# jibo27/3DGS_Hierarchical_Training

Hardware: AMD Instinct MI355X
Metric: train-step images/sec + fwd+bwd ms @1M Gaussians, 980x545; 1/2/4/8 GPU (higher is better)
Workload: dtype f32

## Files before the change

### 3dgs_hierarchical_training_amd/csrc/gsr_kernels.hip

```cpp
#include <hip/hip_runtime.h>
#include <hip/hip_ext.h>
#include <type_traits>
#include <stdint.h>
#include <stdio.h>
#include <string.h>

#include <algorithm>
#include <atomic>
#include <chrono>
#include <cmath>
#include <map>
#include <mutex>
#include <tuple>
#include <vector>

#include "../../include/gsr.h"
#include "gsr_math.h"
#include "adam_math.h"
#include "radix_sort.h"
#include "blend_common.h"

#ifndef GSR_K9_UNROLL
#define GSR_K9_UNROLL 2
#endif
// ... 271 lines not shown
            for (int c = 0; c < 4; c++) {
                s_sh[g * kShStride + col0 + e] = xs[c];
                if (++e == ROW) { e = 0; g++; }
            }
        }
    }
}

template <int ROW, int KN>
__device__ __forceinline__ void stage_store_lin(const float4 (&r)[KN], float* tile, int nG, int tid)
{
    float4* t4 = reinterpret_cast<float4*>(tile);
#pragma unroll
    for (int q = 0; q < stage_regs<ROW>(); q++) {
        const int v = tid + q * kPreThreads;
        if (v < (nG * ROW) / 4) t4[v] = r[q];
    }
}

template <int ROW, int KN>
__device__ __forceinline__ void stage_load_full(float4 (&r)[KN], const float* __restrict__ src, int tid)
{
    static_assert(KN >= stage_regs<ROW>(), "register file too small for the rows");
    constexpr int total4 = kPreThreads * ROW / 4;
    const float4* s4 = reinterpret_cast<const float4*>(src);
#pragma unroll
    for (int q = 0; q < stage_regs<ROW>(); q++) {
        const int v = tid + q * kPreThreads;
        if ((q + 1) * kPreThreads <= total4 || v < total4) r[q] = s4[v];
    }
}
template <int ROW, int KN>
__device__ __forceinline__ void stage_store_lin_full(const float4 (&r)[KN], float* tile, int tid)
{
    constexpr int total4 = kPreThreads * ROW / 4;
    float4* t4 = reinterpret_cast<float4*>(tile);
#pragma unroll
    for (int q = 0; q < stage_regs<ROW>(); q++) {
        const int v = tid + q * kPreThreads;
        if ((q + 1) * kPreThreads <= total4 || v < total4) t4[v] = r[q];
    }
}

__device__ __forceinline__ void count_large_rects(bool act, Splat& s, TileRec& rec, int W, int H, int tiles_x, int tiles_y, int tid)
{
    const int lane = tid & 63;
    for (unsigned long long pm = __ballot(act && s.tiles == kTilesPending); pm != 0ull; pm &= pm - 1ull) {
        const int src = (int)__builtin_ctzll(pm);
        const float bpx = __shfl(s.px, src, 64), bpy = __shfl(s.py, src, 64), bca = __shfl(s.ca, src, 64);
        const float bcb = __shfl(s.cb, src, 64), bcc = __shfl(s.cc, src, 64), bop = __shfl(s.op, src, 64);
        const int brad = __shfl(s.radius, src, 64);
        int x0, y0, x1, y1;
        tile_rect_tight(bpx, bpy, brad, bca, bcb, bcc, bop, W, H, tiles_x, tiles_y, x0, y0, x1, y1);
        const int ww = x1 - x0, full = ww * (y1 - y0);
        const TileTest tt = make_tile_test(bpx, bpy, bca, bcb, bcc, bop);
        uint32_t cnt = 0;
        for (int c0 = 0; c0 < full; c0 += 64) {
            const int c = c0 + lane;
            bool ok = false;
            if (c < full) {
                const int ty = c / ww, tx = c - ty * ww;
                ok = tile_accept(tt, x0 + tx, y0 + ty, W, H);
            }
            cnt += (uint32_t)__popcll(__ballot(ok));
        }
        if (lane == src) { s.tiles = cnt; rec.mask = cnt; }
    }
}

struct DepthHist {
    uint32_t* ghist;
    uint32_t* status;
    uint32_t status_words;
    uint32_t clear_threads;
};

template <int DEG, bool RAW, bool SHO = false>
__global__ __launch_bounds__(kPreThreads) void k_preprocess(CamParams cp, int N, const float* __restrict__ means,
                                                            const float* __restrict__ scales, const float* __restrict__ rots,
                                                            const float* __restrict__ cov_pre, const float* __restrict__ opac,
                                                            const float* __restrict__ shs, const float* __restrict__ shs_rest,
                                                            const float* __restrict__ colors,
                                                            Splat* __restrict__ splat, int32_t* __restrict__ radii,
                                                            uint32_t* __restrict__ dkey, uint32_t* __restrict__ gid,
                                                            TileRec* __restrict__ tilerec, uint32_t* __restrict__ zero_words,
                                                            int zero_count, int block0, DepthHist dh, uint2* __restrict__ early_parts = nullptr,
                                                            uint32_t window_max = 0xffffffffu, uint8_t* __restrict__ visible = nullptr,
                                                            const float* __restrict__ sh_origin = nullptr)
{
    constexpr int NC3 = 3 * (DEG + 1) * (DEG + 1);
    __shared__ float s_sh[kPreThreads * kShStride];
    __shared__ uint32_t s_early[2][kPreThreads / 64];
    const int tid = threadIdx.x;
    const int base = ((int)blockIdx.x + block0) * kPreThreads;
    const int i = base + tid;
    const int model = select_view(cp, (int)blockIdx.x + block0);
    if (blockIdx.x == 0)
        for (int q = tid; q < zero_count; q += kPreThreads) zero_words[q] = 0u;
    constexpr int NR = NC3 > 3 ? NC3 - 3 : 1;
    float4 r_dc[1];
    float4 r_rows[stage_regs<NC3>()];
    bool pend_dc = false, pend_rest = false, pend_full = false;
    const int nG = min(kPreThreads, N - base);
    if (shs) {
        if (shs_rest) {
            const size_t row = (size_t)(cp.M - 1) * 3;
            const float* dc0 = shs + (size_t)base * 3;
            if (vec_ok(dc0, nG * 3)) { stage_load<3>(r_dc, dc0, nG, tid); pend_dc = true; }
            else for (int f = tid; f < nG * 3; f += kPreThreads) s_sh[(f / 3) * kShStride + (f % 3)] = dc0[f];
            if (NC3 > 3) {
                const float* r0 = shs_rest + (size_t)base * row;
                if (row == NR && vec_ok(r0, nG * NR)) { stage_load<NR>(r_rows, r0, nG, tid); pend_rest = true; }
                else for (int f = tid; f < nG * NR; f += kPreThreads) {
                    const int g = f / NR, e = f - g * NR;
                    s_sh[g * kShStride + 3 + e] = shs_rest[(size_t)(base + g) * row + e];
                }
            }
        } else {
            const size_t row = (size_t)cp.M * 3;
            const float* r0 = shs + (size_t)base * row;
            if (row == NC3 && vec_ok(r0, nG * NC3)) { stage_load<NC3>(r_rows, r0, nG, tid); pend_full = true; }
            else for (int f = tid; f < nG * NC3; f += kPreThreads) {
                const int g = f / NC3, e = f - g * NC3;
                s_sh[g * kShStride + e] = shs[(size_t)(base + g) * row + e];
            }
        }
    }
    const bool act = i < N;
    Camera cam = load_camera(cp);
    cam.D = DEG;
    float mean[3] = {0.f, 0.f, 0.f};
    float mraw[3] = {0.f, 0.f, 0.f};
    Splat s;
    TileRec rec;
    uint32_t lo_pack = 0u;
    if (act) {
        mean[0] = means[3 * (size_t)i]; mean[1] = means[3 * (size_t)i + 1]; mean[2] = means[3 * (size_t)i + 2];
        if constexpr (SHO) { mraw[0] = mean[0]; mraw[1] = mean[1]; mraw[2] = mean[2]; }
        apply_points_transform(cp.xf, mean);
        float sc[3] = {0, 0, 0}, rq[4] = {1, 0, 0, 0}, cv[6], colp[3];
        if (cov_pre) {
#pragma unroll
            for (int k = 0; k < 6; k++) cv[k] = cov_pre[6 * (size_t)i + k];
        } else {
#pragma unroll
            for (int k = 0; k < 3; k++) sc[k] = scales[3 * (size_t)i + k];
#pragma unroll
            for (int k = 0; k < 4; k++) rq[k] = rots[4 * (size_t)i + k];
        }
        if (colors) {
#pragma unroll
            for (int k = 0; k < 3; k++) colp[k] = colors[3 * (size_t)i + k];
        }
        float op = opac[i];
        if (RAW) {
            if (!cov_pre) {
#pragma unroll
                for (int k = 0; k < 3; k++) sc[k] = expf(sc[k]);
                const float inv = 1.0f / fmaxf(sqrtf(rq[0] * rq[0] + rq[1] * rq[1] + rq[2] * rq[2] + rq[3] * rq[3]), 1e-12f);
#pragma unroll
                for (int k = 0; k < 4; k++) rq[k] *= inv;
            }
            op = 1.0f / (1.0f + expf(-op));
        }
        preprocess_one(cam, mean, sc, rq, cov_pre ? cv : nullptr, op, nullptr, 3, 1, colors ? colp : nullptr, s, &rec, true, &lo_pack);
    }
    count_large_rects(act, s, rec, cp.W, cp.H, cam.tiles_x, cam.tiles_y, tid);
    rec.rect += (uint32_t)(model * cam.tiles_y) << 12;
    if (early_parts) {
        const uint32_t nt = act ? s.tiles : 0u;
        const uint32_t far = (nt > 0u && __float_as_uint(s.depth) - kDepthKeyBias > window_max) ? 1u : 0u;
        const uint32_t st_ = wave_inclusive_sum(nt), sf_ = wave_inclusive_sum(far);
        if ((tid & 63) == 63) { s_early[0][tid >> 6] = st_; s_early[1][tid >> 6] = sf_; }
        __syncthreads();
        if (tid == 0) {
            uint32_t t0 = 0u, t1 = 0u;
#pragma unroll
            for (int w = 0; w < kPreThreads / 64; w++) { t0 += s_early[0][w]; t1 += s_early[1][w]; }
            early_parts[blockIdx.x + block0] = make_uint2(t0, t1);
        }
    }
    if (shs) {
        constexpr bool kLinOk = NC3 > 3 && (NR & 1);
        const bool lin = kLinOk && pend_dc && pend_rest;
        float* s_dc = s_sh;
        float* s_rest = s_sh + kPreThreads * 3;
        if (lin) {
            stage_store_lin<3>(r_dc, s_dc, nG, tid);
            stage_store_lin<NR>(r_rows, s_rest, nG, tid);
        } else {
            if (pend_dc) stage_store<3>(r_dc, s_sh, 0, nG, tid);
            if (pend_rest) stage_store<NR>(r_rows, s_sh, 3, nG, tid);
            if (pend_full) stage_store<NC3>(r_rows, s_sh, 0, nG, tid);
        }
        __syncthreads();
        if (act && s.radius > 0) {
            float col[3];
            if constexpr (SHO) {
#pragma unroll
                for (int k = 0; k < 3; k++) { cam.cam[k] = sh_origin[k]; mean[k] = mraw[k]; }
            }
            if (lin) splat_sh_color(cam, mean, s_rest + tid * NR - 3, 3, 1, col, s_dc + tid * 3);
            else splat_sh_color(cam, mean, &s_sh[tid * kShStride], 3, 1, col);
            s.r = col[0]; s.g = col[1]; s.b = col[2];
        }
    }
    if (dh.ghist && dh.clear_threads == 0u)
        for (uint32_t q = tid; q < dh.status_words / 4; q += kPreThreads) reinterpret_cast<uint4*>(dh.status)[q] = make_uint4(0u, 0u, 0u, 0u);
    if (!act) return;
    {
        Splat st = s;
        st.tiles = lo_pack;
        splat[i] = st;
    }
    tilerec[i] = rec;
    radii[i] = s.radius;
    if (visible) visible[i] = s.radius > 0 ? 1 : 0;
    const uint32_t key = s.tiles > 0 ? __float_as_uint(s.depth) : 0xffffffffu;
    dkey[i] = key;
    gid[i] = (uint32_t)i;
    if (dh.ghist) {
        const uint32_t x = (uint32_t)i / onesweep_run_len<uint32_t>((uint32_t)N);
#pragma unroll
        for (int p = 0; p < 4; p++) atomicAdd(&dh.ghist[((size_t)p * kOsRanges + x) * 256 + ((key >> (8 * p)) & 255u)], 1u);
    }
}

__global__ __launch_bounds__(256) void k_prepared_begin(int N, const int32_t* __restrict__ radii_in, int32_t* __restrict__ radii_out,
                                                        uint32_t* __restrict__ zero_words, int zero_count)
{
    const int i = blockIdx.x * 256 + threadIdx.x;
    if (i < N) radii_out[i] = radii_in[i];
    if (blockIdx.x == 0)
        for (int q = threadIdx.x; q < zero_count; q += 256) zero_words[q] = 0u;
}

__global__ void k_mark_visible(int N, const float* __restrict__ means, const float* __restrict__ vm, uint8_t* __restrict__ present)
{
    const int i = blockIdx.x * blockDim.x + threadIdx.x;
    if (i >= N) return;
    float v[16];
#pragma unroll
    for (int k = 0; k < 16; k++) v[k] = vm[k];
    present[i] = depth_key(v, means[3 * (size_t)i], means[3 * (size_t)i + 1], means[3 * (size_t)i + 2]) > kNearZ ? 1 : 0;
}

constexpr int kEmitThreads = 256;

__device__ __forceinline__ uint32_t block_inclusive_scan_256(uint32_t v, uint32_t* s_wave , uint32_t& total)
{
    const int lane = threadIdx.x & 63, wave = threadIdx.x >> 6;
    uint32_t x = v;
#pragma unroll
    for (int off = 1; off < 64; off <<= 1) {
        const uint32_t y = __shfl_up(x, off, 64);
        if (lane >= off) x += y;
    }
    if (lane == 63) s_wave[wave] = x;
    __syncthreads();
    uint32_t add = 0;
    for (int w = 0; w < wave; w++) add += s_wave[w];
    total = s_wave[0] + s_wave[1] + s_wave[2] + s_wave[3];
    return x + add;
}

struct ZeroJobs {
    void* p[3];
    uint32_t words[3];
};

__device__ __forceinline__ void scan_report_late(unsigned long long* late_out, unsigned long long all, unsigned long long seq)
{
    __atomic_store_n(late_out, all, __ATOMIC_RELAXED);
    __atomic_store_n(late_out + 2, (unsigned long long)g_onesweep_giveups, __ATOMIC_RELAXED);
    __threadfence_system();
    __atomic_store_n(late_out + 1, seq, __ATOMIC_RELAXED);
    __threadfence_system();
}
template <int NTHR>
__device__ __forceinline__ void block_scan_body(uint32_t* block_sums, int nb, unsigned long long* total_out, const ZeroJobs& zj,
                                                unsigned long long* host_out, unsigned long long host_seq, unsigned long long* s_wsum ,
                                                const unsigned int* window_overflow = nullptr, unsigned long long* late_out = nullptr)
{
    constexpr int NWV = NTHR / 64;
    const int tid = threadIdx.x, lane = tid & 63, wave = tid >> 6;
#pragma unroll
    for (int j = 0; j < 3; j++) {
        uint32_t* z = static_cast<uint32_t*>(zj.p[j]);
        for (uint32_t q = tid; q < zj.words[j]; q += NTHR) z[q] = 0u;
    }
    const int chunk = (nb + NTHR - 1) / NTHR;
    const int lo = min(nb, tid * chunk), hi = min(nb, lo + chunk);
    unsigned long long sum = 0;
    for (int b = lo; b < hi; b++) sum += block_sums[b];
    unsigned long long inc = sum;
#pragma unroll
    for (int off = 1; off < 64; off <<= 1) {
        const unsigned long long y = __shfl_up(inc, off, 64);
        if (lane >= off) inc += y;
    }
    if (lane == 63) s_wsum[wave] = inc;
    __syncthreads();
    unsigned long long add = 0, all = 0;
// ... 1483 lines not shown
        const uint32_t* __restrict__ cur = bb.cur;
        const uint16_t* __restrict__ perm = bb.perm;
        const uint32_t e = cur[0];
        if (table && cur[1 + (blockIdx.x & 7u)]) {
            const int k = (int)perm[blockIdx.x];
            if (k < bb.nslots4) kslot = k;
        }
        if (e < (uint32_t)kVcEntries) cost_out = bb.cost + (size_t)e * bb.items;
    }
}

template <bool REACH>
__global__ __launch_bounds__(64) void k_blend_fwd_w6(int W, int H, int tiles_x, int T, const uint2* __restrict__ ranges,
                                                     const uint32_t* __restrict__ list, const Splat* __restrict__ splat,
                                                     const float* __restrict__ bg, float* __restrict__ out_color,
                                                     float* __restrict__ out_depth, float* __restrict__ out_alpha,
                                                     float* __restrict__ img, uint32_t* __restrict__ staged4, int interleave,
                                                     float* __restrict__ ckpt, int kCkptFirst, int tiles_y, const BlendBalance bb,
                                                     float* __restrict__ out_clamped, const ListCut cut = ListCut{}, const int cut_pass = 0)
{
    if (cut_pass == 2 && cut.ctl[2] == 0u) return;
    __shared__ float4 s_ab[2 * kFwdBufs][64];
    __shared__ float2 s_c[kFwdBufs][64];
    int kslot = (int)(blockIdx.x >> 3);
    uint16_t* cost_out = nullptr;
    blend_fwd_slot(bb, cut_pass != 2, kslot, cost_out);
    blend_fwd_item<REACH>((int)(blockIdx.x & 7), kslot, s_ab, s_c, W, H, tiles_x, T, ranges, list, splat, bg, out_color, out_depth,
                          out_alpha, img, staged4, interleave, ckpt, kCkptFirst, tiles_y, cost_out, out_clamped, cut, cut_pass);
}

template <bool HAS_DA>
__global__ __launch_bounds__(64) void k_blend_fwd_render(int W, int H, int tiles_x, int T, const uint2* __restrict__ ranges,
                                                         const uint32_t* __restrict__ list, const Splat* __restrict__ splat,
                                                         const float* __restrict__ bg, float* __restrict__ out_color,
                                                         float* __restrict__ out_depth, float* __restrict__ out_alpha,
                                                         float* __restrict__, uint32_t* __restrict__, int interleave,
                                                         float* __restrict__, int, int tiles_y, const BlendBalance bb,
                                                         float* __restrict__ out_clamped, const ListCut, const int)
{
    __shared__ float4 s_ab[2 * kFwdBufs][64];
    __shared__ float2 s_c[kFwdBufs][64];
    int kslot = (int)(blockIdx.x >> 3);
    uint16_t* cost_out = nullptr;
    blend_fwd_slot(bb, true, kslot, cost_out);
    blend_fwd_item<true, false, true, HAS_DA>((int)(blockIdx.x & 7), kslot, s_ab, s_c, W, H, tiles_x, T, ranges, list, splat, bg, out_color, out_depth,
                                              out_alpha, nullptr, nullptr, interleave, nullptr, 0, tiles_y, cost_out, out_clamped, ListCut{}, 0);
}

__global__ __launch_bounds__(64) void k_blend_importance(int W, int H, int tiles_x, int T, const uint2* __restrict__ ranges,
                                                         const uint32_t* __restrict__ list, const Splat* __restrict__ splat,
                                                         float* __restrict__ img, uint32_t* __restrict__ staged4, int interleave, int tiles_y,
                                                         const float* __restrict__ color, float* __restrict__ S)
{
    __shared__ float4 s_ab[2 * kFwdBufs][64];
    __shared__ float s_sum[3][64];
    __shared__ uint32_t s_id[64];
    blend_fwd_item<true, true>((int)(blockIdx.x & 7), (int)(blockIdx.x >> 3), s_ab, nullptr, W, H, tiles_x, T, ranges, list, splat, nullptr, nullptr, nullptr,
                               nullptr, img, staged4, interleave, nullptr, 0, tiles_y, nullptr, nullptr, ListCut{}, 0, ImpArgs{color, S, s_sum, s_id});
}

__global__ __launch_bounds__(256) void k_importance_finish(int N, int M, int D, const float* __restrict__ means, const float* __restrict__ xf,
                                                           const float* __restrict__ campos, const float* __restrict__ sh_origin,
                                                           const Splat* __restrict__ splat, const float* __restrict__ S, float* __restrict__ acc)
{
    const int n = (int)blockIdx.x * 16 + (int)(threadIdx.x >> 4), k = (int)(threadIdx.x & 15);
    if (n >= N || k >= (D + 1) * (D + 1)) return;
    const float4 s = reinterpret_cast<const float4*>(S)[n];
    if (s.x == 0.f && s.y == 0.f && s.z == 0.f) return;
    float mean[3] = {means[3 * (size_t)n], means[3 * (size_t)n + 1], means[3 * (size_t)n + 2]};
    float o[3];
    if (sh_origin) { o[0] = sh_origin[0]; o[1] = sh_origin[1]; o[2] = sh_origin[2]; }
    else { apply_points_transform(xf, mean); o[0] = campos[0]; o[1] = campos[1]; o[2] = campos[2]; }
    float basis[16];
    sh_basis_dir(D, mean, o, basis);
    const Splat sp = splat[n];
    const float b = fabsf(basis[k]);
    float* a = acc + ((size_t)n * M + k) * 3;
    if (sp.r > 0.f) a[0] += b * s.x;
    if (sp.g > 0.f) a[1] += b * s.y;
    if (sp.b > 0.f) a[2] += b * s.z;
}


constexpr size_t kItemHdrBytes = 2048;
struct BwdItemHdr {
    uint32_t count[8];
    uint32_t offset[8];
    uint32_t pad[16];
    uint32_t head[8][32];
};
static_assert(sizeof(BwdItemHdr) <= kItemHdrBytes, "item header");
constexpr int kItemBuckets = 32;

__global__ __launch_bounds__(256) void k_bwd_prologue(float4* __restrict__ gg4, size_t n4, const uint32_t* __restrict__ staged4, int T,
                                                      int tiles_x, int interleave, int tpad, int kCkptFirst, int split_ok,
                                                      BwdItemHdr* __restrict__ hdr, uint2* __restrict__ items, uint32_t list_cap,
                                                      uint32_t first_pull, uint32_t* __restrict__ zero_words, int zero_count)
{
    const int tid = threadIdx.x;
    const int builders = hdr ? 8 : 0;
    if ((int)blockIdx.x >= builders) {
        const size_t nblk = gridDim.x - builders, blk = blockIdx.x - builders;
        const float4 z = {0.f, 0.f, 0.f, 0.f};
        for (size_t i = blk * 256 + tid; i < n4; i += nblk * 256) nt_store4(gg4 + i, z);
        return;
    }
    const int x = (int)blockIdx.x;
    if (zero_words && x == 0)
        for (int q = tid; q < zero_count; q += 256) zero_words[q] = 0u;
    __shared__ uint32_t s_cnt[kItemBuckets + 1], s_cur[kItemBuckets];
    if (tid <= kItemBuckets) s_cnt[tid] = 0u;
    if (tid < kItemBuckets) s_cur[tid] = 0u;
    __syncthreads();
    auto items_of = [&](int tile) -> int {
        if (!split_ok) return 1;
        const uint4 sd = *reinterpret_cast<const uint4*>(staged4 + 4 * tile);
        const int nbs = ((int)max(max(sd.x, sd.y), max(sd.z, sd.w)) + 127) / 128;
        if (nbs == 0) return 0;
        return nbs <= kCkptFirst ? 1 : 1 + nbs - kCkptFirst;
    };
    const int slots = tpad >> 3;
    for (int k = tid; k < slots; k += 256) {
        const int tile = slot_tile(interleave, x, k, T, tiles_x);
        if (tile < 0) continue;
        const int ni = items_of(tile);
        for (int q = 0; q < ni; q++) atomicAdd(&s_cnt[min(q, kItemBuckets - 1)], 1u);
    }
    __syncthreads();
    if (tid == 0) {
        uint32_t run = 0;
        for (int q = 0; q < kItemBuckets; q++) { const uint32_t c = s_cnt[q]; s_cnt[q] = run; run += c; }
        s_cnt[kItemBuckets] = run;
        hdr->count[x] = min(run, list_cap); hdr->offset[x] = (uint32_t)x * list_cap; hdr->head[x][0] = first_pull;
    }
    __syncthreads();
    uint2* const mine = items + (size_t)x * list_cap;
    for (int k = tid; k < slots; k += 256) {
        const int tile = slot_tile(interleave, x, k, T, tiles_x);
        if (tile < 0) continue;
        const int ni = items_of(tile);
        for (int q = 0; q < ni; q++) {
            const int bk = min(q, kItemBuckets - 1);
            const uint32_t pos = s_cnt[bk] + atomicAdd(&s_cur[bk], 1u);
            if (pos < list_cap) mine[pos] = make_uint2((uint32_t)tile, (q == 0 ? 0u : (uint32_t)(kCkptFirst + q - 1)) | (ni == 1 ? 0x80000000u : 0u));
        }
    }
}

struct BlendBwdArgs {
    int W, H, tiles_x, tiles_y, T, interleave, kCkptFirst, pad;
    const uint2* ranges;
    const uint32_t* list;
    const Splat* splat;
    const float *bg, *img, *g_color, *g_depth, *g_alpha;
    double* ggrad;
    const float* ckpt;
    float* det_part;
    BwdItemHdr* hdr;
    const uint2* items;
};

#ifdef GSR_K8_PHASES
__device__ unsigned long long g_k8ph[8192 * 8];
#define K8_T(k) do { const unsigned long long now_ = __builtin_readcyclecounter(); k8t[k] += now_ - k8t_last; k8t_last = now_; } while (0)
#else
#define K8_T(k) do { } while (0)
#endif
template <bool HAS_DA>
__global__ __launch_bounds__(128) void k_blend_bwd2(BlendBwdArgs args_)
{
#ifdef GSR_K8_PHASES
    unsigned long long k8t[8] = {0, 0, 0, 0, 0, 0, 0, 0}, k8t_last = __builtin_readcyclecounter();
    k8t[6] = k8t_last;
#endif
    constexpr int NT = 128, NV = HAS_DA ? 10 : 9;
    __shared__ float4 s_ab[2][NT];
    __shared__ typename std::conditional<HAS_DA, float4, float2>::type s_c[NT];
    __shared__ uint32_t s_gid[1][NT];
    __shared__ float s_part[NT][NV];
    uint32_t* const s_max = &s_gid[0][0];
    __shared__ uint32_t s_pull;
    constexpr float kL2E = 1.4426950408889634f, kLn2 = 0.6931471805599453f;
#pragma unroll
    for (int k = 0; k < NV; k++) s_part[threadIdx.x][k] = 0.f;
    int qx = (int)(blockIdx.x & 7u), tried = 0;
    uint32_t qi = blockIdx.x >> 3;
    for (;;) {
#if defined(__HIP_DEVICE_COMPILE__)
    typedef const __attribute__((address_space(4))) BlendBwdArgs* KArgs;
    KArgs ka = (KArgs)__builtin_amdgcn_kernarg_segment_ptr();
    asm volatile("" : "+s"(ka));
    int tid = (int)threadIdx.x;
    asm volatile("" : "+v"(tid));
#else
    const BlendBwdArgs* ka = &args_;
    int tid = (int)threadIdx.x;
#endif
    const int lane = tid & 63, wave = tid >> 6;
    const int part_slot = reduce2_slot<NV>(lane);
    const uint32_t part_off = (uint32_t)(part_slot < 0 ? 0 : part_slot);
    const int W = ka->W, H = ka->H, tiles_x = ka->tiles_x, tiles_y = ka->tiles_y, T = ka->T, kCkptFirst = ka->kCkptFirst;
    BwdItemHdr* const hdr = ka->hdr;
    const uint2* const __restrict__ ranges = ka->ranges;
    const uint32_t* const __restrict__ list = ka->list;
    const Splat* const __restrict__ splat = ka->splat;
    const float* const __restrict__ bg = ka->bg;
    const float* const __restrict__ img = ka->img;
    const float* const __restrict__ g_color = ka->g_color;
    const float* const __restrict__ g_depth = ka->g_depth;
    const float* const __restrict__ g_alpha = ka->g_alpha;
    double* const __restrict__ ggrad = ka->ggrad;
    const float* const __restrict__ ckpt = ka->ckpt;
    float* const __restrict__ det_part = ka->det_part;
    uint32_t qcount = hdr->count[qx];
    while (qi >= qcount) {
        if (++tried == 8) {
#ifdef GSR_K8_PHASES
            const uint32_t w_ = blockIdx.x * 2u + (threadIdx.x >> 6);
            if ((threadIdx.x & 63) == 0 && w_ < 8192u) { k8t[7] = __builtin_readcyclecounter(); for (int q_ = 0; q_ < 8; q_++) g_k8ph[w_ * 8 + q_] = k8t[q_]; }
#endif
            return;
        }
        qx = (qx + 1) & 7;
        qcount = hdr->count[qx];
        qi = 0xffffffffu;
        if (qcount == 0u) continue;
        if (tid == 0) {
            uint32_t v = __hip_atomic_load(&hdr->head[qx][0], __ATOMIC_RELAXED, __HIP_MEMORY_SCOPE_AGENT);
            if (v < qcount) v = __hip_atomic_fetch_add(&hdr->head[qx][0], 1u, __ATOMIC_RELAXED, __HIP_MEMORY_SCOPE_AGENT);
            s_pull = v;
        }
        __syncthreads();
        qi = s_pull;
        __syncthreads();
    }
    const uint2 item = ka->items[hdr->offset[qx] + qi];
    K8_T(0);
#ifdef GSR_K6_TIMING
    const uint32_t dbg_slot = qi < 8192u ? (uint32_t)qx * 8192u + qi : 65536u;
    if (tid == 0 && dbg_slot < 65536) { g_k8_dbg[4 * (size_t)dbg_slot] = wall_clock64(); g_k8_dbg[4 * (size_t)dbg_slot + 1] = 0ull; }
#endif
    const int Tl = tiles_x * tiles_y;
    const size_t Pl = (size_t)W * H, P = Pl * (size_t)(T / Tl);
    const float cyf = 0.5f * (float)H;
    const float bg0 = bg[0], bg1 = bg[1], bg2 = bg[2];
    const int tile = (int)item.x;
    int b0 = (int)(item.y & 0x7fffffffu);
    int b1 = (item.y & 0x80000000u) ? 0x7fffffff : (b0 == 0 ? kCkptFirst : b0 + 1);
    const int bimg = tile / Tl, tl = tile - bimg * Tl;
    const int tx = tl % tiles_x, ty = tl / tiles_x;
    const int px = tx * kTile + (tid & 15);
    const int py0 = ty * kTile + (tid >> 4) * 2;
    const float pxf = (float)(tid & 15);
    const f2 pyf = {(float)((tid >> 4) * 2), (float)((tid >> 4) * 2 + 1)};
    const uint2 rg = ranges[tile];
    const float* const imgb = img + (size_t)bimg * Pl;
    const float* const g_colorb = g_color ? g_color + (size_t)bimg * 3 * Pl : nullptr;
    const float* const g_depthb = g_depth ? g_depth + (size_t)bimg * Pl : nullptr;
    const float* const g_alphab = g_alpha ? g_alpha + (size_t)bimg * Pl : nullptr;
    do {

    const f2 zero2 = {0.f, 0.f};
    f2 Tt = {1.f, 1.f}, S = zero2;
    f2 gC0 = zero2, gC1 = zero2, gC2 = zero2, gD = zero2, gA = zero2;
    uint32_t ncon[2] = {0u, 0u};
#pragma unroll
    for (int p = 0; p < 2; p++) {
// ... 75 lines not shown
    id_nxt = list_at((b0 + 1) * NT + tid);
    for (int b = b0; b < b1; b++) {
        const int buf = 0;
        if (b > b0) __syncthreads();
        if (pend) stage_finish();
        s_ab[0][tid] = ra; s_ab[1][tid] = make_float4(rb.x, rb.y, rb.w, rc.x); s_gid[buf][tid] = rg_id;
        if constexpr (HAS_DA) s_c[tid] = make_float4(rc.y, rc.w, rb.z, 0.f); else s_c[tid] = make_float2(rc.y, rc.w);
        __syncthreads();
        stage_request(id_nxt, (b + 1) * NT + tid < n && b + 1 < b1);
        id_nxt = list_at((b + 2) * NT + tid);
        K8_T(2);
        const int cnt = min(NT, n - b * NT);
        const int cntw = min(cnt, nw - b * NT);
        const uint32_t wbit = 1u << wave;
        const bool r0 = lane < cntw && (__float_as_uint(s_c[lane].y) & wbit);
        const bool r1 = lane + 64 < cntw && (__float_as_uint(s_c[lane + 64].y) & wbit);
        const unsigned long long reach[2] = {__ballot(r0), __ballot(r1)};
#pragma unroll 1
        for (int half = 0; half < 2; half++)
        for (unsigned long long rm = reach[half]; rm != 0ull; rm &= rm - 1ull) {
            const int j = half * 64 + (int)__builtin_ctzll(rm);
            const float4 A = s_ab[0][j], B = s_ab[1][j];
            const auto C = s_c[j];
            const uint32_t idx = (uint32_t)(b * NT + j + 1);
            const float ca = A.z, cb = A.w, cc = B.x, op = B.y, cr = B.z, cg = B.w, cbl = C.x;
            float zd = 0.f;
            if constexpr (HAS_DA) zd = C.z;
            const float dx = A.x - pxf;
            const f2 dy = A.y - pyf;
            const float adx = ca * dx;
            const f2 cdy = cc * dy;
            const f2 p2 = fma2(cdy, dy, fma2(f2{cb, cb}, dy, f2{adx, adx}) * dx);
#if defined(__HIP_DEVICE_COMPILE__)
            f2 G = {__builtin_amdgcn_exp2f(p2.x), __builtin_amdgcn_exp2f(p2.y)};
#else
            f2 G = {exp2f(p2.x), exp2f(p2.y)};
#endif
            f2 alpha = op * G;
            const bool c0p = !(p2.x > 0.f), c0a = !(alpha.x < kAlphaMin), c0n = idx <= ncon[0];
            const bool c1p = !(p2.y > 0.f), c1a = !(alpha.y < kAlphaMin), c1n = idx <= ncon[1];
            const bool v0 = c0p && c0a && c0n, v1 = c1p && c1a && c1n;
            const unsigned long long any01 =
                (__builtin_amdgcn_ballot_w64(c0p) & __builtin_amdgcn_ballot_w64(c0a) & __builtin_amdgcn_ballot_w64(c0n)) |
                (__builtin_amdgcn_ballot_w64(c1p) & __builtin_amdgcn_ballot_w64(c1a) & __builtin_amdgcn_ballot_w64(c1n));
            if (any01 != 0ull) {
                G.x = v0 ? G.x : 0.f; G.y = v1 ? G.y : 0.f;
                alpha = op * G;
                alpha.x = fminf(kAlphaMax, alpha.x); alpha.y = fminf(kAlphaMax, alpha.y);
                const f2 w = alpha * Tt;
                f2 gc = gC0 * cr + gC1 * cg + gC2 * cbl;
                if (HAS_DA) gc += gD * zd + gA;
                S -= gc * w;
                const f2 om = 1.f - alpha;
                const float rab = fast_rcp(om.x * om.y);
                const f2 inv = f2{om.y, om.x} * rab;
                const f2 dLda = gc * Tt - S * inv;
                const f2 dLdpow = G * (op * dLda);
                const f2 t_my = dLdpow * dy;
                float v[10];
                v[0] = (dLdpow.x + dLdpow.y) * dx;
                v[1] = t_my.x + t_my.y;
                v[2] = v[0] * dx;
                v[3] = v[1] * dx;
                v[4] = __builtin_fmaf(t_my.y, dy.y, t_my.x * dy.x);
                v[5] = __builtin_fmaf(G.y, dLda.y, G.x * dLda.x);
                v[6] = __builtin_fmaf(w.y, gC0.y, w.x * gC0.x);
                v[7] = __builtin_fmaf(w.y, gC1.y, w.x * gC1.x);
                v[8] = __builtin_fmaf(w.y, gC2.y, w.x * gC2.x);
                if (HAS_DA) v[9] = __builtin_fmaf(w.y, gD.y, w.x * gD.x);
                Tt *= om;
                const float t = wave_reduce_transposed2<NV>(v, lane);
                uint32_t row;
#if defined(__HIP_DEVICE_COMPILE__)
                asm("s_mul_i32 %0, %1, %2" : "=s"(row) : "s"(j), "n"(NV));
#else
                row = (uint32_t)j * NV;
#endif
                if (part_slot >= 0) atomicAdd(&(&s_part[0][0])[part_off + row], t);
            }
        }
        K8_T(3);
        __syncthreads();
        K8_T(4);
        {
            const int r = tid & 15, q = tid >> 4;
            for (int jj = q; jj < cnt; jj += NT / 16) {
                if (r < NV) {
                    float v = s_part[jj][r];
                    if (r < 2) {
                        const float mo = s_part[jj][r ^ 1];
                        const float cb = s_ab[0][jj].w;
                        const float c2 = 2.f * (r == 0 ? s_ab[0][jj].z : s_ab[1][jj].x);
                        v = fmaf(cb, mo, c2 * v);
                    } else if (r < 5) v *= (r == 3 ? -1.f : -0.5f);
                    __builtin_amdgcn_wave_barrier();
                    s_part[jj][r] = 0.f;
                    if (det_part) det_part[((size_t)rg.x + (size_t)b * NT + jj) * kDetStride + r] = r < 2 ? v * kLn2 : v;
                    else if (v != 0.f) atomicAdd(ggrad + (size_t)s_gid[buf][jj] * kGG + r, (double)(r < 2 ? v * kLn2 : v));
                }
            }
        }
        K8_T(5);
    }
#ifdef GSR_K6_TIMING
    if (threadIdx.x == 0 && dbg_slot < 65536) {
        unsigned long long* d = g_k8_dbg + 4 * (size_t)dbg_slot;
        d[1] = wall_clock64();
        d[2] = ((unsigned long long)__builtin_amdgcn_s_getreg((31 << 11) | 20) << 32) | (unsigned long long)__builtin_amdgcn_s_getreg((31 << 11) | 4);
        d[3] = ((unsigned long long)(uint32_t)n << 32) | (uint32_t)((b1 - b0) * NT);
    }
#endif
    } while (0);
    __syncthreads();
    if (tid == 0) s_pull = __hip_atomic_fetch_add(&hdr->head[qx][0], 1u, __ATOMIC_RELAXED, __HIP_MEMORY_SCOPE_AGENT);
    __syncthreads();
    qi = s_pull;
    tried = 0;
    }
}

template <bool HAS_DA>
__global__ __launch_bounds__(256) void k_blend_bwd1(BlendBwdArgs args_)
{
    constexpr int NT = 128, NTH = 256, NV = HAS_DA ? 10 : 9;
    __shared__ float4 s_ab[2][NT];
    __shared__ typename std::conditional<HAS_DA, float4, float2>::type s_c[NT];
    __shared__ uint32_t s_gid[1][NT];
    __shared__ float s_part[NT][NV];
    uint32_t* const s_max = &s_gid[0][0];
    __shared__ uint32_t s_pull;
    constexpr float kL2E = 1.4426950408889634f, kLn2 = 0.6931471805599453f;
#pragma unroll
    for (int k = 0; k < NV; k++) if (threadIdx.x < NT) s_part[threadIdx.x][k] = 0.f;
    int qx = (int)(blockIdx.x & 7u), tried = 0;
    uint32_t qi = blockIdx.x >> 3;
    for (;;) {
#if defined(__HIP_DEVICE_COMPILE__)
    typedef const __attribute__((address_space(4))) BlendBwdArgs* KArgs;
    KArgs ka = (KArgs)__builtin_amdgcn_kernarg_segment_ptr();
    asm volatile("" : "+s"(ka));
    int tid = (int)threadIdx.x;
    asm volatile("" : "+v"(tid));
#else
    const BlendBwdArgs* ka = &args_;
    int tid = (int)threadIdx.x;
#endif
    const int lane = tid & 63, wave = tid >> 6;
    const int part_slot = reduce2_slot<NV>(lane);
    const uint32_t part_off = (uint32_t)(part_slot < 0 ? 0 : part_slot);
    const int W = ka->W, H = ka->H, tiles_x = ka->tiles_x, tiles_y = ka->tiles_y, T = ka->T, kCkptFirst = ka->kCkptFirst;
    BwdItemHdr* const hdr = ka->hdr;
    const uint2* const __restrict__ ranges = ka->ranges;
    const uint32_t* const __restrict__ list = ka->list;
    const Splat* const __restrict__ splat = ka->splat;
    const float* const __restrict__ bg = ka->bg;
    const float* const __restrict__ img = ka->img;
    const float* const __restrict__ g_color = ka->g_color;
    const float* const __restrict__ g_depth = ka->g_depth;
    const float* const __restrict__ g_alpha = ka->g_alpha;
    double* const __restrict__ ggrad = ka->ggrad;
    const float* const __restrict__ ckpt = ka->ckpt;
    float* const __restrict__ det_part = ka->det_part;
    uint32_t qcount = hdr->count[qx];
    while (qi >= qcount) {
        if (++tried == 8) {
            return;
// ... 137 lines not shown
            const auto C = s_c[j];
            const uint32_t idx = (uint32_t)(b * NT + j + 1);
            const float ca = A.z, cb = A.w, cc = B.x, op = B.y, cr = B.z, cg = B.w, cbl = C.x;
            float zd = 0.f;
            if constexpr (HAS_DA) zd = C.z;
            const float dx = A.x - pxf, dy = A.y - pyf;
            const float p2 = __builtin_fmaf(cc * dy, dy, __builtin_fmaf(cb, dy, ca * dx) * dx);
#if defined(__HIP_DEVICE_COMPILE__)
            float G = __builtin_amdgcn_exp2f(p2);
#else
            float G = exp2f(p2);
#endif
            float alpha = op * G;
            const bool c0p = !(p2 > 0.f), c0a = !(alpha < kAlphaMin), c0n = idx <= ncon;
            const bool v0 = c0p && c0a && c0n;
            const unsigned long long any0 = __builtin_amdgcn_ballot_w64(c0p) & __builtin_amdgcn_ballot_w64(c0a) & __builtin_amdgcn_ballot_w64(c0n);
            if (any0 != 0ull) {
                G = v0 ? G : 0.f;
                alpha = fminf(kAlphaMax, op * G);
                const float w = alpha * Tt;
                float gc = gC0 * cr + gC1 * cg + gC2 * cbl;
                if (HAS_DA) gc += gD * zd + gA;
                S -= gc * w;
                const float om = 1.f - alpha;
                const float dLda = gc * Tt - S * fast_rcp(om);
                const float dLdpow = G * (op * dLda);
                const float t_my = dLdpow * dy;
                float v[10];
                v[0] = dLdpow * dx;
                v[1] = t_my;
                v[2] = v[0] * dx;
                v[3] = t_my * dx;
                v[4] = t_my * dy;
                v[5] = G * dLda;
                v[6] = w * gC0;
                v[7] = w * gC1;
                v[8] = w * gC2;
                if (HAS_DA) v[9] = w * gD;
                Tt *= om;
                const float t = wave_reduce_transposed2<NV>(v, lane);
                uint32_t row;
#if defined(__HIP_DEVICE_COMPILE__)
                asm("s_mul_i32 %0, %1, %2" : "=s"(row) : "s"(j), "n"(NV));
#else
                row = (uint32_t)j * NV;
#endif
                if (part_slot >= 0) atomicAdd(&(&s_part[0][0])[part_off + row], t);
            }
        }
        __syncthreads();
        {
            const int r = tid & 15, q = tid >> 4;
            for (int jj = q; jj < cnt; jj += NTH / 16) {
                if (r < NV) {
                    float v = s_part[jj][r];
                    if (r < 2) {
                        const float mo = s_part[jj][r ^ 1];
                        const float cb = s_ab[0][jj].w;
                        const float c2 = 2.f * (r == 0 ? s_ab[0][jj].z : s_ab[1][jj].x);
                        v = fmaf(cb, mo, c2 * v);
                    } else if (r < 5) v *= (r == 3 ? -1.f : -0.5f);
                    __builtin_amdgcn_wave_barrier();
                    s_part[jj][r] = 0.f;
                    if (det_part) det_part[((size_t)rg.x + (size_t)b * NT + jj) * kDetStride + r] = r < 2 ? v * kLn2 : v;
                    else if (v != 0.f) atomicAdd(ggrad + (size_t)s_gid[buf][jj] * kGG + r, (double)(r < 2 ? v * kLn2 : v));
                }
            }
        }
    }
    } while (0);
    __syncthreads();
    if (tid == 0) s_pull = __hip_atomic_fetch_add(&hdr->head[qx][0], 1u, __ATOMIC_RELAXED, __HIP_MEMORY_SCOPE_AGENT);
    __syncthreads();
    qi = s_pull;
    tried = 0;
    }
}

struct PrepOut {
    CamParams cp;
    Splat* splat;
    int32_t* radii;
    uint32_t* dkey;
    uint32_t* gid;
    TileRec* rec;
    DepthHist dh;
    uint2* early_parts;
    uint32_t early_window;
};

struct DensDev {
    const int32_t* radii;
    float *grad_accum, *denom, *max_radii;
};

struct AdamDev {
    float* m[6];
    float* v[6];
    float step_size[6];
    float b1, b2, eps;
    float inv_bc2s[6];
    long long dp[6], dm[6], dv[6];
};
template <typename T>
__device__ __forceinline__ T* adam_out(T* p, long long d) { return reinterpret_cast<T*>(reinterpret_cast<char*>(p) + d); }

__device__ __forceinline__ void adam_rows(const float* s_g, int stride, int col0, int row, int nact, float* __restrict__ p,
                                          float* __restrict__ m, float* __restrict__ v, int nG, int tid, float step_size, float bc2,
                                          int grp, const AdamDev& ad)
{
    const int total = nG * row;
    float* const po = adam_out(p, ad.dp[grp]); float* const mo = adam_out(m, ad.dm[grp]); float* const vo = adam_out(v, ad.dv[grp]);
    if (((((uintptr_t)p | (uintptr_t)m | (uintptr_t)v | (uintptr_t)po | (uintptr_t)mo | (uintptr_t)vo) & 15) == 0) && (total & 3) == 0) {
        float4* p4 = reinterpret_cast<float4*>(p);
        float4* m4 = reinterpret_cast<float4*>(m);
        float4* v4 = reinterpret_cast<float4*>(v);
        float4* po4 = reinterpret_cast<float4*>(po);
        float4* mo4 = reinterpret_cast<float4*>(mo);
        float4* vo4 = reinterpret_cast<float4*>(vo);
        for (int q = tid; q < total / 4; q += kPreThreads) {
            float4 pp = p4[q], mm = nt_load4(m4 + q), vv = nt_load4(v4 + q);
            const int f = 4 * q;
            int g = f / row, e = f - g * row;
            float gs[4];
#pragma unroll
            for (int c = 0; c < 4; c++) {
                gs[c] = e < nact ? s_g[g * stride + col0 + e] : 0.f;
                if (++e == row) { e = 0; g++; }
            }
            adam_one(pp.x, gs[0], mm.x, vv.x, ad.b1, ad.b2, ad.eps, step_size, bc2);
            adam_one(pp.y, gs[1], mm.y, vv.y, ad.b1, ad.b2, ad.eps, step_size, bc2);
            adam_one(pp.z, gs[2], mm.z, vv.z, ad.b1, ad.b2, ad.eps, step_size, bc2);
            adam_one(pp.w, gs[3], mm.w, vv.w, ad.b1, ad.b2, ad.eps, step_size, bc2);
            nt_store4(po4 + q, pp); nt_store4(mo4 + q, mm); nt_store4(vo4 + q, vv);
        }
    } else {
        for (int f = tid; f < total; f += kPreThreads) {
            const int g = f / row, e = f - g * row;
            float pp = p[f], mm = m[f], vv = v[f];
            adam_one(pp, e < nact ? s_g[g * stride + col0 + e] : 0.f, mm, vv, ad.b1, ad.b2, ad.eps, step_size, bc2);
            po[f] = pp; mo[f] = mm; vo[f] = vv;
        }
    }
}

constexpr int kAdamPrefetch = GSR_K9_PREFETCH;
template <bool KEEP, int KP = 0>
__device__ __forceinline__ void adam_rows_lin(float* s_g, int total, float* __restrict__ p, float* __restrict__ m,
                                              float* __restrict__ v, int tid, float step_size, float bc2, int grp, const AdamDev& ad,
                                              const float4* pm = nullptr, const float4* pv = nullptr)
{
    float4* p4 = reinterpret_cast<float4*>(p);
    float4* m4 = reinterpret_cast<float4*>(m);
    float4* v4 = reinterpret_cast<float4*>(v);
    float4* g4 = reinterpret_cast<float4*>(s_g);
    float* const po = adam_out(p, ad.dp[grp]); float* const mo = adam_out(m, ad.dm[grp]); float* const vo = adam_out(v, ad.dv[grp]);
    float4* po4 = reinterpret_cast<float4*>(po);
    float4* mo4 = reinterpret_cast<float4*>(mo);
    float4* vo4 = reinterpret_cast<float4*>(vo);
    if ((((uintptr_t)m | (uintptr_t)v | (uintptr_t)po | (uintptr_t)mo | (uintptr_t)vo) & 15) == 0) {
        int q0 = tid;
        if constexpr (KP > 0) {
#pragma unroll
            for (int k = 0; k < KP; k++) {
                const int q = tid + k * kPreThreads;
                if (q < total / 4) {
                    float4 pp = p4[q], mm = pm[k], vv = pv[k];
// ... 453 lines not shown
                    float4* g4 = reinterpret_cast<float4*>(s_dc);
                    const float4 g = g4[tid];
                    adam_one(dP.x, g.x, dM.x, dV.x, ad.b1, ad.b2, ad.eps, ad.step_size[1], ad.inv_bc2s[1]);
                    adam_one(dP.y, g.y, dM.y, dV.y, ad.b1, ad.b2, ad.eps, ad.step_size[1], ad.inv_bc2s[1]);
                    adam_one(dP.z, g.z, dM.z, dV.z, ad.b1, ad.b2, ad.eps, ad.step_size[1], ad.inv_bc2s[1]);
                    adam_one(dP.w, g.w, dM.w, dV.w, ad.b1, ad.b2, ad.eps, ad.step_size[1], ad.inv_bc2s[1]);
                    nt_store4(reinterpret_cast<float4*>(adam_out(pd, ad.dp[1])) + tid, dP);
                    nt_store4(reinterpret_cast<float4*>(adam_out(ad.m[1] + b * 3, ad.dm[1])) + tid, dM);
                    nt_store4(reinterpret_cast<float4*>(adam_out(ad.v[1] + b * 3, ad.dv[1])) + tid, dV);
                    if (PREP >= 0) g4[tid] = dP;
                }
            } else {
            adam_rows_lin<(PREP >= 0)>(s_dc, nG * 3, const_cast<float*>(shs) + b * 3, ad.m[1] + b * 3, ad.v[1] + b * 3, tid, ad.step_size[1], ad.inv_bc2s[1], 1, ad);
            if (DEG > 0 || ad.m[2]) {
                if (kAdamPrefetch > 0 && pf_ok)
                    adam_rows_lin<(PREP >= 0), kAdamPrefetch>(s_rest, nG * NRL, const_cast<float*>(shs_rest) + b * NRL, ad.m[2] + b * NRL, ad.v[2] + b * NRL, tid,
                                                              ad.step_size[2], ad.inv_bc2s[2], 2, ad, pf_m, pf_v);
                else
                    adam_rows_lin<(PREP >= 0)>(s_rest, nG * NRL, const_cast<float*>(shs_rest) + b * NRL, ad.m[2] + b * NRL, ad.v[2] + b * NRL, tid, ad.step_size[2], ad.inv_bc2s[2], 2, ad);
            }
            }
            if (i < N) {
                const size_t gi = (size_t)i;
                adam_own_apply<3>(const_cast<float*>(means) + 3 * gi, ad.m[0] + 3 * gi, ad.v[0] + 3 * gi, om_mean, own_g, ad.step_size[0], ad.inv_bc2s[0], 0, ad, PREP >= 0 ? nmean : nullptr);
                adam_own_apply<1>(const_cast<float*>(opac_raw) + gi, ad.m[3] + gi, ad.v[3] + gi, om_op, own_g + 3, ad.step_size[3], ad.inv_bc2s[3], 3, ad, PREP >= 0 ? &nop : nullptr);
                adam_own_apply<3>(const_cast<float*>(scales) + 3 * gi, ad.m[4] + 3 * gi, ad.v[4] + 3 * gi, om_sc, own_g + 4, ad.step_size[4], ad.inv_bc2s[4], 4, ad, PREP >= 0 ? nsc : nullptr);
                adam_own_apply<4>(const_cast<float*>(rots) + 4 * gi, ad.m[5] + 4 * gi, ad.v[5] + 4 * gi, om_rq, own_g + 7, ad.step_size[5], ad.inv_bc2s[5], 5, ad, PREP >= 0 ? nrq : nullptr);
                if (ds.radii && e_rad > 0) {
                    ds.max_radii[i] = fmaxf(e_ds[0], (float)e_rad);
                    ds.grad_accum[i] = e_ds[1] + e_m2dn;
                    ds.denom[i] = e_ds[2] + 1.f;
                }
            }
            K9_T(3);
            if (PREP < 0) { K9_T_FLUSH(); return; }
            lds_barrier();
            const bool act = i < N;
            const int model2 = select_view(po.cp, (int)blockIdx.x);
            Camera cam2 = load_camera(po.cp);
            cam2.D = PREP < 0 ? 0 : PREP;
            Splat s2;
            TileRec rec2;
            uint32_t lo2 = 0u;
            float mean2[3] = {nmean[0], nmean[1], nmean[2]};
            if (act) {
                apply_points_transform(po.cp.xf, mean2);
                float sc2[3], rq2[4] = {nrq[0], nrq[1], nrq[2], nrq[3]};
#pragma unroll
                for (int k = 0; k < 3; k++) sc2[k] = expf(nsc[k]);
                const float inv = 1.0f / fmaxf(sqrtf(rq2[0] * rq2[0] + rq2[1] * rq2[1] + rq2[2] * rq2[2] + rq2[3] * rq2[3]), 1e-12f);
#pragma unroll
                for (int k = 0; k < 4; k++) rq2[k] *= inv;
                const float op2 = 1.0f / (1.0f + expf(-nop));
                preprocess_one(cam2, mean2, sc2, rq2, nullptr, op2, nullptr, 3, 1, nullptr, s2, &rec2, true, &lo2);
            }
            count_large_rects(act, s2, rec2, po.cp.W, po.cp.H, cam2.tiles_x, cam2.tiles_y, tid);
            rec2.rect += (uint32_t)(model2 * cam2.tiles_y) << 12;
            if (po.early_parts) {
                __shared__ uint32_t s_early2[2][kPreThreads / 64];
                const uint32_t nt = act ? s2.tiles : 0u;
                const uint32_t far = (nt > 0u && __float_as_uint(s2.depth) - kDepthKeyBias > po.early_window) ? 1u : 0u;
                const uint32_t st_ = wave_inclusive_sum(nt), sf_ = wave_inclusive_sum(far);
                if ((tid & 63) == 63) { s_early2[0][tid >> 6] = st_; s_early2[1][tid >> 6] = sf_; }
                lds_barrier();
                if (tid == 0) {
                    uint32_t t0 = 0u, t1 = 0u;
#pragma unroll
                    for (int w = 0; w < kPreThreads / 64; w++) { t0 += s_early2[0][w]; t1 += s_early2[1][w]; }
                    po.early_parts[blockIdx.x] = make_uint2(t0, t1);
                }
            }
            if (act && s2.radius > 0) {
                float col[3];
                splat_sh_color(cam2, mean2, s_rest + tid * NRL - 3, 3, 1, col, s_dc + tid * 3);
                s2.r = col[0]; s2.g = col[1]; s2.b = col[2];
            }
            uint32_t key2 = 0xffffffffu;
            if (act) {
                { Splat st = s2; st.tiles = lo2; po.splat[i] = st; }
                po.rec[i] = rec2;
                po.radii[i] = s2.radius;
                key2 = s2.tiles > 0 ? __float_as_uint(s2.depth) : 0xffffffffu;
                po.dkey[i] = key2;
                po.gid[i] = (uint32_t)i;
            }
            K9_T(4);
            if (po.dh.ghist) {
                lds_barrier();
                uint32_t* h = reinterpret_cast<uint32_t*>(s_sh);
#pragma unroll
                for (int q = 0; q < 1024 / kPreThreads; q++) h[q * kPreThreads + tid] = 0u;
                lds_barrier();
                if (act) {
#pragma unroll
                    for (int p = 0; p < 4; p++) atomicAdd(&h[p * 256 + ((key2 >> (8 * p)) & 255u)], 1u);
                }
                lds_barrier();
                const uint32_t x = (uint32_t)base / onesweep_run_len<uint32_t>((uint32_t)N);
#pragma unroll
                for (int q = 0; q < 1024 / kPreThreads; q++) {
                    const int e = q * kPreThreads + tid;
                    const uint32_t c = h[e];
                    if (c) atomicAdd(&po.dh.ghist[((size_t)(e >> 8) * kOsRanges + x) * 256 + (e & 255)], c);
                }
                for (uint32_t q = blockIdx.x * kPreThreads + tid; q < po.dh.status_words / 4; q += po.dh.clear_threads)
                    reinterpret_cast<uint4*>(po.dh.status)[q] = make_uint4(0u, 0u, 0u, 0u);
            }
            K9_T(5);
            K9_T_FLUSH();
            return;
        }
        if (i < N) {
            const size_t gi = (size_t)i;
            adam_own_apply<3>(const_cast<float*>(means) + 3 * gi, ad.m[0] + 3 * gi, ad.v[0] + 3 * gi, om_mean, own_g, ad.step_size[0], ad.inv_bc2s[0], 0, ad, PREP >= 0 ? nmean : nullptr);
            adam_own_apply<1>(const_cast<float*>(opac_raw) + gi, ad.m[3] + gi, ad.v[3] + gi, om_op, own_g + 3, ad.step_size[3], ad.inv_bc2s[3], 3, ad, PREP >= 0 ? &nop : nullptr);
            adam_own_apply<3>(const_cast<float*>(scales) + 3 * gi, ad.m[4] + 3 * gi, ad.v[4] + 3 * gi, om_sc, own_g + 4, ad.step_size[4], ad.inv_bc2s[4], 4, ad, PREP >= 0 ? nsc : nullptr);
            adam_own_apply<4>(const_cast<float*>(rots) + 4 * gi, ad.m[5] + 4 * gi, ad.v[5] + 4 * gi, om_rq, own_g + 7, ad.step_size[5], ad.inv_bc2s[5], 5, ad, PREP >= 0 ? nrq : nullptr);
            if (ds.radii && e_rad > 0) {
                ds.max_radii[i] = fmaxf(e_ds[0], (float)e_rad);
                ds.grad_accum[i] = e_ds[1] + e_m2dn;
                ds.denom[i] = e_ds[2] + 1.f;
            }
        }
        adam_rows(s_sh, kShStride, 0, 3, 3, const_cast<float*>(shs) + b * 3, ad.m[1] + b * 3, ad.v[1] + b * 3, nG, tid, ad.step_size[1], ad.inv_bc2s[1], 1, ad);
        if (DEG == 0 && !ad.m[2]) {}
        else if (rrow == 45 && NC3 == 48)
            adam_rows(s_sh, kShStride, 3, 45, 45, const_cast<float*>(shs_rest) + b * 45, ad.m[2] + b * 45, ad.v[2] + b * 45, nG, tid, ad.step_size[2], ad.inv_bc2s[2], 2, ad);
        else if (rrow > 0)
            adam_rows(s_sh, kShStride, 3, rrow, NC3 - 3, const_cast<float*>(shs_rest) + b * rrow, ad.m[2] + b * rrow, ad.v[2] + b * rrow, nG, tid,
                      ad.step_size[2], ad.inv_bc2s[2], 2, ad);
    } else if (lin && d_shs && d_shs_rest) {
        __syncthreads();
        stage_out_lin<3>(s_dc, d_shs + (size_t)base * 3, nG, tid);
        stage_out_lin<NRL>(s_rest, d_shs_rest + (size_t)base * NRL, nG, tid);
    } else if (shs && d_shs) {
        __syncthreads();
        const int row = cp.M * 3;
        if (d_shs_rest) {
            const int rrow = row - 3;
            float* dc0 = d_shs + (size_t)base * 3;
            if (vec_ok(dc0, nG * 3)) stage_out_vec<3>(s_sh, 0, dc0, nG, tid);
            else for (int f = tid; f < nG * 3; f += kPreThreads) dc0[f] = s_sh[(f / 3) * kShStride + (f % 3)];
            if (rrow == NC3 - 3) {
                constexpr int NR = NC3 > 3 ? NC3 - 3 : 1;
                float* r0 = d_shs_rest + (size_t)base * NR;
                if (NC3 > 3 && vec_ok(r0, nG * NR)) stage_out_vec<NR>(s_sh, 3, r0, nG, tid);
                else for (int f = tid; f < nG * NR; f += kPreThreads) r0[f] = s_sh[(f / NR) * kShStride + 3 + (f % NR)];
            } else {
                for (int f = tid; f < nG * rrow; f += kPreThreads) {
                    const int g = f / rrow, e = f - g * rrow + 3;
                    d_shs_rest[(size_t)(base + g) * rrow + (e - 3)] = e < NC3 ? s_sh[g * kShStride + e] : 0.f;
                }
            }
        } else if (row == NC3) {
            float* r0 = d_shs + (size_t)base * NC3;
            if (vec_ok(r0, nG * NC3)) stage_out_vec<NC3>(s_sh, 0, r0, nG, tid);
            else for (int f = tid; f < nG * NC3; f += kPreThreads) r0[f] = s_sh[(f / NC3) * kShStride + (f % NC3)];
        } else {
            for (int f = tid; f < nG * row; f += kPreThreads) {
                const int g = f / row, e = f - g * row;
                d_shs[(size_t)(base + g) * row + e] = e < NC3 ? s_sh[g * kShStride + e] : 0.f;
            }
        }
    }
}

__global__ __launch_bounds__(256) void k_det_iota(uint32_t R, uint32_t* __restrict__ pos, const uint32_t* __restrict__ list, uint32_t* __restrict__ ids,
                                                  uint32_t n_gaussians)
{
    const uint32_t i = blockIdx.x * 256u + threadIdx.x;
    if (i < R) { pos[i] = i; ids[i] = min(list[i], n_gaussians - 1u); }
}
__global__ __launch_bounds__(256) void k_det_reduce(uint32_t R, const uint32_t* __restrict__ gid_sorted, const uint32_t* __restrict__ pos_sorted,
                                                    const float* __restrict__ part, double* __restrict__ ggrad)
{
    const uint32_t i = blockIdx.x * 256u + threadIdx.x;
    if (i >= R) return;
    const uint32_t g = gid_sorted[i];
    if (i > 0 && gid_sorted[i - 1] == g) return;
    double acc[kDetStride];
#pragma unroll
    for (int r = 0; r < kDetStride; r++) acc[r] = 0.0;
    for (uint32_t j = i; j < R && gid_sorted[j] == g; j++) {
        const float* p = part + (size_t)pos_sorted[j] * kDetStride;
#pragma unroll
        for (int r = 0; r < kDetStride; r++) acc[r] += (double)p[r];
    }
#pragma unroll
    for (int r = 0; r < kDetStride; r++) ggrad[(size_t)g * kGG + r] = acc[r];
}

__global__ __launch_bounds__(256) void k_cam_reduce(const float* __restrict__ partial, int nblocks, float* __restrict__ d_vm,
                                                    float* __restrict__ d_pm, float* __restrict__ d_campos, float* __restrict__ d_xf,
                                                    BatchDev bt)
{
    __shared__ double s[256];
    const int q = blockIdx.x, m = blockIdx.y;
    int lo = 0, hi = nblocks;
    if (bt.B > 1) {
#pragma unroll
        for (int k = 0; k < kMaxBatch; k++)
            if (k == m) { lo = bt.first_block[k]; hi = min(nblocks, bt.first_block[k + 1]); }
        if (d_vm) d_vm += 16 * m;
        if (d_pm) d_pm += 16 * m;
        if (d_campos) d_campos += 3 * m;
        if (d_xf) d_xf += 12 * m;
    }
    double a = 0;
    for (int b = lo + threadIdx.x; b < hi; b += 256) a += partial[(size_t)b * kCamVals + q];
    s[threadIdx.x] = a;
    __syncthreads();
    for (int off = 128; off > 0; off >>= 1) {
        if (threadIdx.x < off) s[threadIdx.x] += s[threadIdx.x + off];
        __syncthreads();
    }
    if (threadIdx.x == 0) {
        const float v = (float)s[0];
        if (q < 16) { if (d_vm) d_vm[q] = v; }
        else if (q < 32) { if (d_pm) d_pm[q - 16] = v; }
        else if (q < 35) { if (d_campos) d_campos[q - 32] = v; }
        else if (d_xf) d_xf[q - 35] = v;
    }
}

struct GeomLayout {
    size_t splat;
    size_t total;
};
static GeomLayout geom_layout(int32_t N)
{
    GeomLayout g;
    g.splat = 0;
    g.total = align256((size_t)(N > 0 ? N : 1) * sizeof(Splat));
    return g;
}

struct PrepLayout {
    size_t splat, radii, dkey, gid, rec, sort, early, bytes;
};
static PrepLayout prep_layout(int32_t N)
{
    const size_t n = (size_t)(N > 0 ? N : 1);
    PrepLayout p;
    size_t o = 0;
    p.splat = o; o += align256(n * sizeof(Splat));
    p.radii = o; o += align256(n * 4);
    p.dkey = o; o += align256(n * 4);
    p.gid = o; o += align256(n * 4);
    p.rec = o; o += align256(n * sizeof(TileRec));
    p.sort = o; o += align256(onesweep_scratch_bytes((uint32_t)n));
    p.early = o; o += align256(((n + kPreThreads - 1) / kPreThreads) * sizeof(uint2));
    p.bytes = o;
    return p;
}

struct FwdScratch {
    size_t dkey, gid, dkey_alt, gid_alt, ntiles, srec, block_sums, total, early, sort;
    size_t bytes;
};
static FwdScratch fwd_scratch_layout(int32_t N)
{
    const size_t n = (size_t)(N > 0 ? N : 1);
    FwdScratch s;
    size_t o = 0;
    s.dkey = o; o += align256(n * 4);
    s.gid = o; o += align256(n * 4);
    s.dkey_alt = o; o += align256(n * 4);
    s.gid_alt = o; o += align256(n * 4);
    s.ntiles = o; o += align256(n * sizeof(TileRec));
    s.srec = o; o += align256(n * sizeof(TileRec));
    s.block_sums = o; o += align256(((n + kEmitThreads - 1) / kEmitThreads) * 4);
    s.total = o; o += 256;
    s.early = o; o += align256(((n + kPreThreads - 1) / kPreThreads) * sizeof(uint2));
    s.sort = o; o += radix_scratch_bytes((uint32_t)n);
    s.bytes = o;
    return s;
}

struct BinLayout {
    size_t list, ranges, ckpt, items, bytes;
};

static size_t bwd_list_cap(int64_t R, size_t T) { return ((size_t)(R > 0 ? R : 0) >> 7) + T + 8; }
static BinLayout bin_layout(int64_t R, int32_t W, int32_t H, int32_t B = 1)
{
    const size_t T = (size_t)((W + kTile - 1) / kTile) * ((H + kTile - 1) / kTile) * (size_t)(B > 1 ? B : 1);
    BinLayout b;
    b.ranges = 0;
    b.list = align256((T ? T : 1) * sizeof(uint2));
    b.ckpt = b.list + align256((size_t)(R > 0 ? R : 1) * 4);
    b.items = b.ckpt + align256((((size_t)(R > 0 ? R : 0) >> 7) + T + 1) * kCkptFloats * sizeof(float));
    b.bytes = b.items + kItemHdrBytes + align256(8 * bwd_list_cap(R, T) * sizeof(uint2));
    return b;
}

struct BinScratch {
    size_t tile, tile_alt, gid_alt, sort, bytes;
};
static BinScratch bin_scratch_layout(int64_t R, int key_bytes = 4)
{
    const size_t r = (size_t)(R > 0 ? R : 1);
    BinScratch s;
    size_t o = 0;
    s.tile = o; o += align256(r * (size_t)key_bytes);
    s.tile_alt = o; o += align256(r * (size_t)key_bytes);
    s.gid_alt = o; o += align256(r * 4);
    s.sort = o; o += radix_scratch_bytes((uint32_t)r);
    s.bytes = o;
    return s;
}

struct ViewCostCache { int dev, W, H, map, items; uint8_t* mem; size_t bytes; };
static std::vector<ViewCostCache> g_view_costs;
static std::map<std::tuple<int, int, int, int>, bool> g_full_depth_sort;

struct PinSlot { unsigned long long* host = nullptr; unsigned long long* dev = nullptr; bool busy = false;
                 unsigned long long seq = 0;
                 bool pending = false; unsigned long long pending_seq = 0, pending_R = 0, pending_giveups = 0; };
static std::mutex g_state_mutex;
static std::map<int, std::vector<PinSlot*>> g_pin_slots;
static std::map<std::tuple<int, int, int, int>, uint64_t> g_hints;
static long long g_hint_override = -1;
static int g_speculate = 1;
static int g_deterministic = 0;
static int g_bwd_split = 0;
static int g_ckpt_first = 1;
static int g_depth_sort9 = 1;
static int g_tile_sort = 1;
static int g_tile_sort_emit_max_n = 400000;
static int g_tile_sort_max_avg = 700;
static int g_direct_bin = 1;
static int g_view_pose_tol_e6 = 2000;
static int g_list_cut = 1;
static int g_list_cut_min_n = 2000000;
static int g_list_cut_margin_e3 = 50;
static int g_list_cut_deep = 8;
static int g_early_r = 1;
static int g_blend_balance = 1;
static int g_tile_map = 2;
static std::atomic<long long> g_spec_overflows{0}, g_spec_forwards{0}, g_exact_forwards{0}, g_depth_window_resorts{0};
static std::atomic<long long> g_fwd_calls{0}, g_fwd_ns{0}, g_fwd_wait_ns{0}, g_bwd_calls{0}, g_bwd_ns{0}, g_frozen_bwd_calls{0};
struct CallTimer {
    std::atomic<long long>&calls, &ns;
    std::chrono::steady_clock::time_point t0 = std::chrono::steady_clock::now();
    CallTimer(std::atomic<long long>& c, std::atomic<long long>& n) : calls(c), ns(n) {}
    ~CallTimer() { calls++; ns += std::chrono::duration_cast<std::chrono::nanoseconds>(std::chrono::steady_clock::now() - t0).count(); }
};

static int n_bucket(int N) { return N > 0 ? (int)std::floor(2.0 * std::log2((double)N)) : 0; }

static PinSlot* acquire_pin_slot(int dev)
{
    std::lock_guard<std::mutex> lk(g_state_mutex);
    auto& v = g_pin_slots[dev];
    for (PinSlot* s : v)
        if (!s->busy) { s->busy = true; return s; }
    PinSlot* s = new PinSlot();
    if (hipHostMalloc((void**)&s->host, 64, hipHostMallocMapped) != hipSuccess ||
        hipHostGetDevicePointer((void**)&s->dev, s->host, 0) != hipSuccess) { delete s; return nullptr; }
    s->host[0] = 0; s->host[1] = 0;
    for (int q = 4; q < 8; q++) s->host[q] = 0;
    s->busy = true;
    v.push_back(s);
    return s;
}
static std::atomic<long long> g_late_checks{0}, g_late_mismatches{0};
static int g_debug_late_bias = 0;
static int late_check(PinSlot* s, bool wait, unsigned long long* got_total, unsigned long long* want_total)
{
    if (!s->pending) return 0;
    volatile unsigned long long* hp = s->host;
    if (hp[5] != s->pending_seq) {
        if (!wait) return 0;
        const auto limit = std::chrono::steady_clock::now() + std::chrono::milliseconds(200);
        while (hp[5] != s->pending_seq && std::chrono::steady_clock::now() < limit) cpu_relax();
        if (hp[5] != s->pending_seq) { (void)hipDeviceSynchronize(); }
        if (hp[5] != s->pending_seq) { s->pending = false; return 0; }
    }
    std::atomic_thread_fence(std::memory_order_acquire);
    s->pending = false;
    g_late_checks++;
    *got_total = hp[4]; *want_total = s->pending_R;
    if (hp[4] != s->pending_R || hp[6] != s->pending_giveups) { g_late_mismatches++; return 1; }
    return 0;
}
struct PinLease {
    PinSlot* s;
    explicit PinLease(PinSlot* s_) : s(s_) {}
    ~PinLease() { if (s) { std::lock_guard<std::mutex> lk(g_state_mutex); s->busy = false; } }
};

static inline int64_t pack_fwd_flags(int ppt, int tile_map, int ckpt_first)
{
    return 1 | ((int64_t)ppt << 1) | ((int64_t)tile_map << 4) | ((int64_t)ckpt_first << 6) | ((int64_t)(ppt >= 5) << 13);
}

static int batch_dev(const GsrBatch* bt, int32_t N, int32_t H, BatchDev& out)
{
    out = BatchDev{};
    out.B = 1;
    if (!bt || bt->B <= 1) return GSR_OK;
    if (bt->B > kMaxBatch || !bt->first_block) return fail(GSR_ERR_ARG, "batch: 2..16 models and a first_block table expected%s");
    const int nblocks = (N + kPreThreads - 1) / kPreThreads;
    if (bt->first_block[0] != 0 || bt->first_block[bt->B] != nblocks || (N % kPreThreads) != 0)
        return fail(GSR_ERR_ARG, "batch: first_block must run from 0 to N / 128 and N must be a multiple of 128 (pad every model)%s");
    for (int q = 0; q < bt->B; q++)
        if (bt->first_block[q + 1] < bt->first_block[q]) return fail(GSR_ERR_ARG, "batch: first_block must be non-decreasing%s");
    if ((long long)bt->B * ((H + kTile - 1) / kTile) > 4095) return fail(GSR_ERR_RANGE, "batch: more than 4095 tile rows in total%s");
    out.B = bt->B;
    for (int q = 0; q <= bt->B; q++) out.first_block[q] = bt->first_block[q];
    for (int q = bt->B + 1; q <= kMaxBatch; q++) out.first_block[q] = nblocks;
    return GSR_OK;
}

static int check_common(int32_t N, int32_t M, int32_t D, int32_t W, int32_t H)
{
    if (N < 0 || W <= 0 || H <= 0) return fail(GSR_ERR_ARG, "bad sizes%s");
    if (D < 0 || D > 3) return fail(GSR_ERR_ARG, "sh_degree must be 0..3%s");
    if (M < 0 || M > 16) return fail(GSR_ERR_ARG, "at most 16 SH coefficients per Gaussian%s");
    if (W > 4095 * kTile || H > 4095 * kTile) return fail(GSR_ERR_RANGE, "image side longer than 65520 pixels%s");
    return GSR_OK;
}

}
// ... 19 lines not shown
}
size_t gsr_image_bytes(int32_t W, int32_t H) { return gsr_image_bytes_batched(W, H, 1); }

int gsr_profile_read(const char* name, double* total_ms, int64_t* count)
{
    if (!name || !total_ms || !count) return GSR_ERR_ARG;
    for (int id = 0; id < P_COUNT; id++) {
        if (strcmp(name, kProfNames[id])) continue;
        std::lock_guard<std::mutex> lk(g_prof_mutex);
        double tot = 0; int64_t n = 0;
        for (auto& p : g_prof_events[id]) {
            float ms = 0.f;
            if (hipEventSynchronize(p.b) == hipSuccess && hipEventElapsedTime(&ms, p.a, p.b) == hipSuccess) { tot += ms; n++; }
            (void)hipEventDestroy(p.a); (void)hipEventDestroy(p.b);
        }
        g_prof_events[id].clear();
        *total_ms = tot; *count = n;
        return GSR_OK;
    }
    return GSR_ERR_ARG;
}
size_t gsr_forward_scratch_bytes(int32_t N) { return fwd_scratch_layout(N).bytes; }
size_t gsr_binning_bytes(int64_t R, int32_t W, int32_t H) { return bin_layout(R, W, H).bytes; }
size_t gsr_binning_scratch_bytes(int64_t R) { return bin_scratch_layout(R).bytes; }
size_t gsr_backward_scratch_bytes(int32_t N)
{
    const size_t n = (size_t)(N > 0 ? N : 1);
    return align256(n * kGG * sizeof(double)) + align256(((n + kPreThreads - 1) / kPreThreads) * kCamVals * 4);
}
size_t gsr_sort_scratch_bytes(uint32_t n) { return radix_scratch_bytes(n); }
size_t gsr_prepared_bytes(int32_t N) { return prep_layout(N).bytes; }
size_t gsr_prepared_radii_offset(int32_t N) { return prep_layout(N).radii; }
int gsr_prepare_supported(int32_t M, int32_t D, int32_t raw_params) { return (raw_params && M == 16 && D >= 0 && D <= 3) ? 1 : 0; }
const char* gsr_last_error(void) { return g_err; }
int gsr_version(void) { return 116; }
size_t gsr_struct_bytes(int32_t which)
{
    return which == 0 ? sizeof(GsrForwardArgs) : which == 1 ? sizeof(GsrBackwardArgs) : which == 2 ? sizeof(GsrForwardOut) : 0;
}

#ifdef GSR_K8_PHASES
int gsr_debug_k8_phases(unsigned long long* host_dst) { return (int)hipMemcpyFromSymbol(host_dst, HIP_SYMBOL(g_k8ph), sizeof(unsigned long long) * 8 * 8192); }
#endif
#ifdef GSR_OS_TIMING
int gsr_debug_os_timing(unsigned long long* host_dst) { return (int)hipMemcpyFromSymbol(host_dst, HIP_SYMBOL(g_os_dbg), sizeof(unsigned long long) * 8 * 4096); }
int gsr_debug_gh_timing(unsigned long long* host_dst) { return (int)hipMemcpyFromSymbol(host_dst, HIP_SYMBOL(g_gh_dbg), sizeof(unsigned long long) * 8 * 512); }
#endif
#ifdef GSR_K9_TIMING
int gsr_debug_k9_timing(unsigned long long* host_dst, int reset)
{
    (void)reset;
    return (int)hipMemcpyFromSymbol(host_dst, HIP_SYMBOL(g_k9_dbg), sizeof(unsigned long long) * 8 * kK9DbgWaves);
}
#endif
#ifdef GSR_DB_TIMING
int gsr_debug_db_timing(unsigned long long* host_dst) { return (int)hipMemcpyFromSymbol(host_dst, HIP_SYMBOL(g_db_dbg), sizeof(unsigned long long) * 16); }
#endif
#ifdef GSR_K6_TIMING
int gsr_debug_k6_timing(unsigned long long* host_dst, int blocks)
{
    return (int)hipMemcpyFromSymbol(host_dst, HIP_SYMBOL(g_k6_dbg), sizeof(unsigned long long) * 4 * (size_t)blocks);
}
int gsr_debug_k6_counts(uint32_t* host_dst, int blocks)
{
    return (int)hipMemcpyFromSymbol(host_dst, HIP_SYMBOL(g_k6_cnt), sizeof(uint32_t) * 2 * (size_t)blocks);
}
int gsr_debug_k6_cycles(unsigned long long* host_dst, int blocks)
{
    return (int)hipMemcpyFromSymbol(host_dst, HIP_SYMBOL(g_k6_cyc), sizeof(unsigned long long) * 2 * (size_t)blocks);
}
int gsr_debug_k8_timing(unsigned long long* host_dst, int blocks)
{
    return (int)hipMemcpyFromSymbol(host_dst, HIP_SYMBOL(g_k8_dbg), sizeof(unsigned long long) * 4 * (size_t)blocks);
}
#endif
int gsr_set_option(const char* name, int value)
{
    if (!name) return GSR_ERR_ARG;
    if (!strcmp(name, "blend_fwd_ppt")) {
        if (value != 0 && value != 6 && value != 7) return GSR_ERR_ARG;
        g_blend_ppt = value; return GSR_OK;
    }
    if (!strcmp(name, "ab_variants")) return 0;
    if (!strcmp(name, "bwd_split")) { if (value < 0 || value > 64) return GSR_ERR_ARG; g_bwd_split = value; return GSR_OK; }
    if (!strcmp(name, "ckpt_first")) { if (value < 1 || value > 64) return GSR_ERR_ARG; g_ckpt_first = value; return GSR_OK; }
    if (!strcmp(name, "tile_map")) { if (value < 0 || value > 2) return GSR_ERR_ARG; g_tile_map = value; return GSR_OK; }
    if (!strcmp(name, "blend_balance")) { g_blend_balance = value ? 1 : 0; return GSR_OK; }
    if (!strcmp(name, "early_r")) { g_early_r = value ? 1 : 0; return GSR_OK; }
    if (!strcmp(name, "list_cut")) { g_list_cut = value < 0 || value > 2 ? 1 : value; return GSR_OK; }
    if (!strcmp(name, "list_cut_min_n")) { g_list_cut_min_n = value < 0 ? 2000000 : value; return GSR_OK; }
    if (!strcmp(name, "view_cache_reset")) {
        int dev_id = 0;
        if (hipGetDevice(&dev_id) != hipSuccess || hipDeviceSynchronize() != hipSuccess) return GSR_ERR_HIP;
        std::lock_guard<std::mutex> lk(g_state_mutex);
        for (auto& c : g_view_costs)
            if (c.dev == dev_id && hipMemset(c.mem, 0, c.bytes) != hipSuccess) return GSR_ERR_HIP;
        return GSR_OK;
    }
    if (!strcmp(name, "list_cut_margin_e3")) { g_list_cut_margin_e3 = value < 0 ? 50 : value; return GSR_OK; }
    if (!strcmp(name, "list_cut_deep")) { g_list_cut_deep = value < 0 ? 8 : value; return GSR_OK; }
    if (!strcmp(name, "debug_late_bias")) { g_debug_late_bias = value; return GSR_OK; }
    if (!strcmp(name, "tile_sort")) { if (value < 0 || value > 2) return GSR_ERR_ARG; g_tile_sort = value; return GSR_OK; }
    if (!strcmp(name, "tile_sort_max_avg")) { if (value < 0) return GSR_ERR_ARG; g_tile_sort_max_avg = value; return GSR_OK; }
    if (!strcmp(name, "view_pose_tol_e6")) { if (value < 0) return GSR_ERR_ARG; g_view_pose_tol_e6 = value; return GSR_OK; }
    if (!strcmp(name, "depth_sort9")) { g_depth_sort9 = value ? 1 : 0; return GSR_OK; }
    if (!strcmp(name, "direct_binning")) { g_direct_bin = value ? 1 : 0; return GSR_OK; }
    if (!strcmp(name, "speculative_binning")) { g_speculate = value ? 1 : 0; return GSR_OK; }
    if (!strcmp(name, "deterministic_backward")) { g_deterministic = value ? 1 : 0; return GSR_OK; }
    if (!strcmp(name, "binning_capacity_hint")) {
        std::lock_guard<std::mutex> lk(g_state_mutex);
        g_hint_override = value > 0 ? value : -1;
        return GSR_OK;
    }
    if (!strcmp(name, "reset_speculation")) {
        std::lock_guard<std::mutex> lk(g_state_mutex);
        g_hints.clear(); g_hint_override = -1;
        g_spec_overflows = 0; g_spec_forwards = 0; g_exact_forwards = 0; g_depth_window_resorts = 0;
        g_full_depth_sort.clear();
        return GSR_OK;
    }
    if (!strcmp(name, "profile")) { g_profile = (value == 2 || value == 3) ? value : (value ? 1 : 0); g_profile_tick = 0; return GSR_OK; }
    if (!strcmp(name, "prep_hist_max_n")) { g_prep_hist_max_n = value; return GSR_OK; }
    if (!strcmp(name, "small_sort9")) { if (value < 0) return GSR_ERR_ARG; g_small_sort9 = value; return GSR_OK; }
    if (!strcmp(name, "poll_iters")) { g_poll_iters = value < 0 ? 0 : value; return GSR_OK; }
    if (!strcmp(name, "emit_hist")) { g_emit_hist = value ? 1 : 0; return GSR_OK; }
    if (!strcmp(name, "sort_algo")) { if (value < 0 || value > 2) return GSR_ERR_ARG; g_sort_algo = value; return GSR_OK; }
    if (!strcmp(name, "blend_bwd_ppt")) {
        if (value < 0 || value > 2) return GSR_ERR_ARG;
        g_bwd_ppt = value; return GSR_OK;
    }
    return GSR_ERR_ARG;
}

struct DirectBinScratch { size_t M, GT, tbase, bsum, cut_chunk, cut_tend, cut_flag, cut_ctl, cut_bkey, cut_hist, bytes; };
static bool direct_bin_geometry(int N, int T, DirectBin& db, DirectBinScratch& ds)
{
    if (N < 1 || T < 1 || T > kDbMaxTiles) return false;
    static std::atomic<int> cus_cached{0};
    int cus = cus_cached.load(std::memory_order_relaxed);
    if (!cus) {
        int dev = 0, n = 0;
        cus = (hipGetDevice(&dev) == hipSuccess && hipDeviceGetAttribute(&n, hipDeviceAttributeMultiprocessorCount, dev) == hipSuccess && n > 0) ? n : 256;
        cus_cached.store(cus, std::memory_order_relaxed);
    }
    db.N = N; db.T = T; db.Tp = (T + 63) & ~63;
    const int lds = 12 * db.Tp + 4 * kDbPairs;
    const int per_cu = std::min(16, (160 * 1024) / lds);
    const long long resident = std::max<long long>(1, (long long)cus * per_cu);
    const int min_s = 128;
    long long S = ((long long)N + resident - 1) / resident;
    S = std::max<long long>(min_s, (S + 63) & ~63ll);
    if (S > 65472) return false;
    db.S = (int)S;
    db.NC = (int)(((long long)N + S - 1) / S);
    int G = 1;
    while (G * G < db.NC) G++;
    db.Cg = std::max(1, std::min((db.NC + G - 1) / G, 65535 / db.S));
    db.G = (db.NC + db.Cg - 1) / db.Cg;
    if (db.G > kDbMaxGroups) return false;
    size_t o = 0;
    ds.M = o; o += align256((size_t)db.NC * db.Tp * sizeof(uint16_t));
    ds.GT = o; o += align256((size_t)db.G * db.Tp * sizeof(uint32_t));
    ds.tbase = o; o += align256((size_t)(db.Tp + 1) * sizeof(uint32_t));
    ds.bsum = o; o += align256((size_t)db.G * ((db.Tp + 255) / 256) * sizeof(uint32_t));
    ds.cut_chunk = o; o += align256((size_t)db.Tp * sizeof(uint16_t));
    ds.cut_tend = o; o += align256((size_t)db.Tp * sizeof(uint32_t));
// ... 202 lines not shown
                                   a->out_color, ro_depth, ro_alpha, img, staged, opt_map, ckpt, opt_ckpt, tiles_y, BlendBalance{}, a->out_color_clamped);
        }
        if (ppt == 7 && lc.key && lc_capacity > 0) {
            ProfScope ps(P_CUT_REPAIR, st);
            const int per = (db.NC + 7) / 8, grid = std::max(8 * per, (T + 63) / 64);
            hipLaunchKernelGGL((k_chunk_scatter<false, 2>), dim3(grid), dim3(64), (size_t)12 * db.Tp + 4 * kDbPairs, st, db, W, H,
                               tiles_x, tiles_y, sorted_gid, reinterpret_cast<const TileRec*>(fs + L.srec), splat, list, ranges,
                               (uint32_t)std::min<uint64_t>(lc_capacity, 0xffffffffull), (const uint32_t*)nullptr, (uint2*)nullptr, lc);
            hipLaunchKernelGGL(k_blend_fwd_w6<true>, dim3(8 * 4 * slots_per_xcd(opt_map, T, tiles_x)), dim3(64), 0, st, W, H, tiles_x, T, ranges, list, splat, a->bg,
                               a->out_color, a->out_depth, a->out_alpha, img, staged, opt_map, ckpt, opt_ckpt, tiles_y, bb, a->out_color_clamped, lc, 2);
        }
        GSR_HIP(hipGetLastError());
        return GSR_OK;
    };

    if (N == 0) {
        rc = ro_workspace();
        if (rc) return rc;
        rc = alloc_binning(0);
        if (rc) return rc;
        rc = launch_binning(0, nullptr, false);
        if (rc) return rc;
        rc = launch_blend(false);
        if (rc) return rc;
        if (!ro) { out->binning = bin; out->binning_bytes = B.bytes; }
        return GSR_OK;
    }

    if (!a->means3D || !a->opacities || (!ro && !a->geom) || !a->radii || !a->viewmatrix || !a->projmatrix)
        return fail(GSR_ERR_ARG, "missing input pointer%s");
    if ((a->shs == nullptr) == (a->colors_precomp == nullptr)) return fail(GSR_ERR_ARG, "provide exactly one of shs / colors_precomp%s");
    if ((a->cov3D_precomp == nullptr) == (a->scales == nullptr || a->rotations == nullptr))
        return fail(GSR_ERR_ARG, "provide exactly one of (scales, rotations) / cov3D_precomp%s");
    if (a->shs && (!a->campos || a->M < (a->D + 1) * (a->D + 1))) return fail(GSR_ERR_ARG, "shs needs campos and M >= (D+1)^2%s");
    rc = ro_workspace();
    if (rc) return rc;

    int dev_id = 0;
    GSR_HIP(hipGetDevice(&dev_id));
    const auto hint_key = std::make_tuple(dev_id, W, H * NB, n_bucket(N));
    uint64_t hint = 0;
    {
        std::lock_guard<std::mutex> lk(g_state_mutex);
        if (g_hint_override > 0) { hint = (uint64_t)g_hint_override; g_hint_override = -1; }
        else { auto it = g_hints.find(hint_key); if (it != g_hints.end()) hint = it->second; }
    }
    const bool speculative = g_speculate && g_sort_algo == 2 && hint > 0;
    const uint64_t cap = speculative ? hint : 0;
    {
        const int ts_mode = g_tile_sort;
        const uint64_t avg = (hint > 0 ? hint : (uint64_t)N * 4u) / (uint64_t)T;
        const bool auto_ok = ts_mode == 1 && avg <= (uint64_t)g_tile_sort_max_avg && (direct || N / std::max(1, NB) <= g_tile_sort_emit_max_n);
        tsort = (ts_mode == 2 || auto_ok) && g_sort_algo == 2 && (direct ? NB == 1 : true);
    }

    fs = static_cast<uint8_t*>(a->alloc(align256(L.bytes) + (direct ? dbs.bytes : 0), GSR_ALLOC_SCRATCH, a->alloc_user));
    if (!fs) return fail(GSR_ERR_ALLOC, "scratch allocation failed%s");
    if (speculative) {
        rc = alloc_binning(cap);
        if (rc) return rc;
    }
    uint32_t* dkey = reinterpret_cast<uint32_t*>(fs + L.dkey);
    uint32_t* gid = reinterpret_cast<uint32_t*>(fs + L.gid);
    uint32_t* dkey_alt = reinterpret_cast<uint32_t*>(fs + L.dkey_alt);
    uint32_t* gid_alt = reinterpret_cast<uint32_t*>(fs + L.gid_alt);
    TileRec* ntiles = reinterpret_cast<TileRec*>(fs + L.ntiles);
    uint32_t* block_sums = reinterpret_cast<uint32_t*>(fs + L.block_sums);
    unsigned long long* total = reinterpret_cast<unsigned long long*>(fs + L.total);
    const bool depth_onesweep = g_sort_algo != 0;
    CamParams cp = {a->viewmatrix, a->projmatrix, a->campos, a->tanfovx, a->tanfovy, a->scale_modifier, W, H, a->D, a->M, a->points_transform, bt};
    const int grid = (N + kPreThreads - 1) / kPreThreads;
    uint32_t* zero_words = depth_onesweep ? reinterpret_cast<uint32_t*>(fs + L.sort) : nullptr;
    const int zero_count = depth_onesweep ? (int)kOnesweepHeadWordsMax : 0;
    uint8_t* depth_scratch = fs + L.sort;
    bool depth_hist_done = false;
    const bool early_r = g_early_r && speculative && depth_onesweep;
    uint2* early_parts = early_r ? reinterpret_cast<uint2*>(a->prepared ? static_cast<uint8_t*>(a->prepared) + prep_layout(N).early : fs + L.early) : nullptr;
    const uint32_t early_window = (N > g_prep_hist_max_n || (g_small_sort9 && !a->prepared && N >= g_small_sort9)) ? (1u << 27) - 1u : 0xffffffffu;
    if (a->prepared) {
        if (a->prepared != a->geom) return fail(GSR_ERR_ARG, "prepared: geom must be the prepared buffer itself%s");
        const PrepLayout PL = prep_layout(N);
        uint8_t* pb = static_cast<uint8_t*>(a->prepared);
        dkey = reinterpret_cast<uint32_t*>(pb + PL.dkey);
        gid = reinterpret_cast<uint32_t*>(pb + PL.gid);
        ntiles = reinterpret_cast<TileRec*>(pb + PL.rec);
        ProfScope ps(P_PRE_FWD, st);
        if (depth_onesweep) { depth_scratch = pb + PL.sort; depth_hist_done = prep_counts_digits(N); }
        if (a->radii != reinterpret_cast<const int32_t*>(pb + PL.radii))
            hipLaunchKernelGGL(k_prepared_begin, dim3((N + 255) / 256), dim3(256), 0, st, N, reinterpret_cast<const int32_t*>(pb + PL.radii),
                               a->radii, (uint32_t*)nullptr, 0);
    } else {
#define GSR_PRE_(DEG, RAW, SHO)                                                                                                     \
    hipLaunchKernelGGL((k_preprocess<DEG, RAW, SHO>), dim3(grid), dim3(kPreThreads), 0, st, cp, N, a->means3D, a->scales,           \
                       a->rotations, a->cov3D_precomp, a->opacities, a->shs, a->shs_rest, a->colors_precomp, splat, a->radii, dkey, gid, \
                       ntiles, zero_words, zero_count, 0, DepthHist{}, early_parts, early_window, a->visible, a->sh_origin)
#define GSR_PRE(DEG) do { if (a->raw_params) GSR_PRE_(DEG, true, false); else GSR_PRE_(DEG, false, false); } while (0)
#define GSR_PRE_SHO(DEG) do { if (a->raw_params) GSR_PRE_(DEG, true, true); else GSR_PRE_(DEG, false, true); } while (0)
    {
        ProfScope ps(P_PRE_FWD, st);
        if (a->sh_origin) {
            switch (a->D) {
                case 0: GSR_PRE(0); break;
                case 1: GSR_PRE_SHO(1); break;
                case 2: GSR_PRE_SHO(2); break;
                default: GSR_PRE_SHO(3); break;
            }
        } else {
        switch (a->shs ? a->D : 0) {
            case 0: GSR_PRE(0); break;
            case 1: GSR_PRE(1); break;
            case 2: GSR_PRE(2); break;
            default: GSR_PRE(3); break;
        }
        }
    }
#undef GSR_PRE_SHO
#undef GSR_PRE
#undef GSR_PRE_
    }
    int in_alt = 0;
    bool wide_depth = depth_onesweep && g_depth_sort9 && !depth_hist_done && (N > g_prep_hist_max_n || (g_small_sort9 && N >= g_small_sort9));
    if (wide_depth) {
        std::lock_guard<std::mutex> lk(g_state_mutex);
        auto it = g_full_depth_sort.find(hint_key);
        if (it != g_full_depth_sort.end() && it->second) wide_depth = false;
    }
    const unsigned int* window_overflow = wide_depth ? onesweep_overflow_word(depth_scratch) : nullptr;
    if (tsort) wide_depth = false;
    const unsigned int* window_overflow_ = tsort ? nullptr : window_overflow;
    PinLease pin(acquire_pin_slot(dev_id));
    if (!pin.s) return fail(GSR_ERR_HIP, "pinned read-back slot allocation failed%s");
    {
        unsigned long long got = 0, want = 0;
        if (late_check(pin.s, true, &got, &want)) {
            char msg[200];
            snprintf(msg, sizeof msg, "a PREVIOUS forward's binning was invalid: early instance count %llu, its scan counted %llu (or a sort look-back gave up)%%s", want, got);
            return fail(GSR_ERR_HIP, msg);
        }
    }
    OsRider rider = {};
    if (early_r) { rider.parts = early_parts; rider.nparts = (uint32_t)grid; rider.host = pin.s->dev; rider.seq = ++pin.s->seq; }
    ts_rec = ntiles; ts_dkey = dkey;
    if (!tsort) {
        ProfScope ps(P_SORT_DEPTH, st);
        GSR_HIP(depth_onesweep ? onesweep_sort_pairs<uint32_t>(dkey, gid, dkey_alt, gid_alt, (uint32_t)N, 0, wide_depth ? 27 : 32, depth_scratch, &in_alt, st,
                                                               nullptr, true, depth_hist_done, wide_depth ? 9 : 8, kDepthKeyBias, early_r ? &rider : nullptr)
                               : radix_sort_pairs<uint32_t>(dkey, gid, dkey_alt, gid_alt, (uint32_t)N, 0, 32, fs + L.sort, &in_alt, st));
    }
    sorted_gid = tsort ? nullptr : (in_alt ? gid_alt : gid);
    auto launch_counts = [&](const BlendBalance& bal, const ZeroJobs& zjobs, const unsigned int* wo, unsigned long long seq, bool publish = true) {
        TileRec* srec = reinterpret_cast<TileRec*>(fs + L.srec);
        unsigned long long* const host_slot = publish ? pin.s->dev : nullptr;
        unsigned long long* const late_slot = publish ? nullptr : pin.s->dev + 4;
        if (direct) {
            hipLaunchKernelGGL(k_chunk_counts, dim3(db.NC + (bal.hdr ? 8 : 0)), dim3(kEmitThreads), (size_t)2 * db.Tp, st, db, W, H,
                               tiles_x, tiles_y, sorted_gid, ntiles, splat, tsort ? (TileRec*)nullptr : srec, bal,
                               (tsort && early_r && !publish) ? rider : OsRider{}, lc);
            hipLaunchKernelGGL(k_chunk_scan1, dim3((db.Tp + 255) / 256, db.G), dim3(256), 0, st, db);
            hipLaunchKernelGGL(k_chunk_scan2, dim3((db.Tp + 255) / 256), dim3(256), lc.key ? (size_t)db.NC * 4 : 0, st, db, total, zjobs, host_slot, seq, wo,
                               late_slot, lc);
        } else {
            hipLaunchKernelGGL(k_tile_counts, dim3(nb + (bal.hdr ? 8 : 0)), dim3(kEmitThreads), 0, st, N, sorted_gid, ntiles, block_sums,
                               tsort ? (TileRec*)nullptr : srec, bal, nb, (tsort && early_r && !publish) ? rider : OsRider{});
            hipLaunchKernelGGL(k_block_scan, dim3(1), dim3(1024), 0, st, block_sums, nb, total, zjobs, host_slot, seq, wo, late_slot);
        }
    };
    {
        ProfScope ps(P_SCAN, st);
        ZeroJobs zj = {};
        if (speculative) {
            zj.p[0] = ranges; zj.words[0] = (uint32_t)((size_t)T * sizeof(uint2) / 4);
            zj.p[1] = staged; zj.words[1] = (uint32_t)T * 4u;
            if (bs) { zj.p[2] = bs + S.sort; zj.words[2] = kOnesweepHeadWords; }
        }
        {
            const int nslots4 = 4 * slots_per_xcd(opt_map, T, tiles_x), items = 8 * nslots4;
            if (g_blend_balance && NB == 1 && opt_ppt == 7 && items <= 65535 && nslots4 <= 20 * kEmitThreads && a->viewmatrix) {
                const size_t hdr_bytes = align256(sizeof(ViewCostHdr));
                const size_t vc_cut = align256(hdr_bytes + (size_t)kVcEntries * items * sizeof(uint16_t));
                const size_t vc_own = vc_cut + align256((size_t)kVcEntries * T * sizeof(uint32_t));
                const size_t vc_bytes = vc_own + align256((size_t)kVcEntries * sizeof(uint32_t));
                uint8_t* mem = nullptr;
                {
                    std::lock_guard<std::mutex> lk(g_state_mutex);
                    for (auto& c : g_view_costs)
                        if (c.dev == dev_id && c.W == W && c.H == H && c.map == opt_map && c.items == items) mem = c.mem;
                    if (!mem && g_view_costs.size() < 64) {
                        if (hipMalloc((void**)&mem, vc_bytes) == hipSuccess) {
                            if (hipMemset(mem, 0, vc_bytes) == hipSuccess) {
                                g_view_costs.push_back({dev_id, W, H, opt_map, items, mem, vc_bytes});
                            } else {
                                (void)hipGetLastError();
                                (void)hipFree(mem);
                                mem = nullptr;
                            }
                        } else {
                            (void)hipGetLastError();
                            mem = nullptr;
                        }
                    }
                }
                if (mem) {
                    uint8_t* ib = img_base + balance_off;
                    bb.hdr = reinterpret_cast<ViewCostHdr*>(mem);
                    bb.cost = reinterpret_cast<uint16_t*>(mem + hdr_bytes);
                    bb.cur = reinterpret_cast<uint32_t*>(ib);
                    bb.perm = reinterpret_cast<uint16_t*>(ib + 256);
                    bb.vm = a->viewmatrix; bb.pt = a->points_transform; bb.view_id = (long long)a->view_id;
                    bb.tol = 1e-6f * (float)g_view_pose_tol_e6;
                    bb.items = items; bb.nslots4 = nslots4; bb.W = W; bb.H = H;
                    if (!ro && direct && !tsort && db.NC <= 16000 && T == db.T && (g_list_cut == 2 || (g_list_cut == 1 && N >= g_list_cut_min_n))) {
                        uint8_t* dm = fs + align256(L.bytes);
                        lc.key = reinterpret_cast<uint32_t*>(mem + vc_cut);
                        lc.owner_n = reinterpret_cast<uint32_t*>(mem + vc_own);
                        lc.stats = &bb.hdr->pad[2];
                        lc.cur = bb.cur;
                        lc.chunk = reinterpret_cast<uint16_t*>(dm + dbs.cut_chunk);
                        lc.tend = reinterpret_cast<uint32_t*>(dm + dbs.cut_tend);
                        lc.flag = reinterpret_cast<uint32_t*>(dm + dbs.cut_flag);
                        lc.ctl = reinterpret_cast<uint32_t*>(dm + dbs.cut_ctl);
                        lc.bkey = reinterpret_cast<uint32_t*>(dm + dbs.cut_bkey);
                        lc.hist = reinterpret_cast<uint32_t*>(dm + dbs.cut_hist);
                        lc.skey = in_alt ? dkey_alt : dkey;
                        lc.tbase = reinterpret_cast<uint32_t*>(dm + dbs.tbase);
                        lc.margin = 1e-3f * (float)g_list_cut_margin_e3;
                        lc.dmax = std::max(0, g_list_cut_deep);
                    }
                }
            }
        }
        if (direct) {
            uint8_t* dm = fs + align256(L.bytes);
            db.M = reinterpret_cast<uint16_t*>(dm + dbs.M); db.GT = reinterpret_cast<uint32_t*>(dm + dbs.GT); db.tbase = reinterpret_cast<uint32_t*>(dm + dbs.tbase);
            db.bsum = reinterpret_cast<uint32_t*>(dm + dbs.bsum);
            zj.p[0] = nullptr; zj.words[0] = 0u;
            zj.p[2] = nullptr; zj.words[2] = 0u;
        }
        if (early_r) launch_counts(bb, zj, window_overflow_, rider.seq, false);
        else launch_counts(bb, zj, window_overflow_, ++pin.s->seq);
    }
    GSR_HIP(hipGetLastError());

    if (speculative) {
        rc = launch_binning(cap, total, true);
        if (rc) return rc;
        rc = launch_blend(true);
        if (rc) return rc;
        {
            const auto w0 = std::chrono::steady_clock::now();
            volatile unsigned long long* hp = pin.s->host;
            const unsigned long long want = pin.s->seq;
            bool seen = false;
            if (g_poll_iters > 0) {
                const auto limit = w0 + std::chrono::nanoseconds((long long)g_poll_iters * 50);
                while (!(seen = (hp[1] == want))) {
                    for (int it = 0; it < 64 && !(seen = (hp[1] == want)); it++) cpu_relax();
                    if (seen || std::chrono::steady_clock::now() > limit) break;
                }
            }
            if (!seen) GSR_HIP(hipStreamSynchronize(st));
            std::atomic_thread_fence(std::memory_order_acquire);
            g_fwd_wait_ns += std::chrono::duration_cast<std::chrono::nanoseconds>(std::chrono::steady_clock::now() - w0).count();
        }
        g_spec_forwards++;
    } else {
        const auto w0 = std::chrono::steady_clock::now();
        GSR_HIP(hipStreamSynchronize(st));
        g_fwd_wait_ns += std::chrono::duration_cast<std::chrono::nanoseconds>(std::chrono::steady_clock::now() - w0).count();
        g_exact_forwards++;
    }
    R = *static_cast<volatile unsigned long long*>(pin.s->host);
    {
        static std::map<int, unsigned long long> seen_giveups;
        const unsigned long long gv = static_cast<volatile unsigned long long*>(pin.s->host)[2];
        bool fresh;
        {
            std::lock_guard<std::mutex> lk(g_state_mutex);
            unsigned long long& seen = seen_giveups[dev_id];
            fresh = gv != seen;
            seen = gv;
        }
        if (fresh)
            return fail(GSR_ERR_HIP, "a radix-sort look-back gave up (status words overwritten?): the binning of this or the previous forward is invalid%s");
        if (early_r) {
            pin.s->pending = true; pin.s->pending_seq = rider.seq; pin.s->pending_R = R + (unsigned long long)g_debug_late_bias; pin.s->pending_giveups = gv;
            g_debug_late_bias = 0;
        }
    }
    bool resorted = false;
    if (wide_depth && static_cast<volatile unsigned long long*>(pin.s->host)[3] != 0ull) {
        { std::lock_guard<std::mutex> lk(g_state_mutex); g_full_depth_sort[hint_key] = true; }
        g_depth_window_resorts++;
        uint32_t *k0 = in_alt ? dkey_alt : dkey, *v0 = in_alt ? gid_alt : gid, *k1 = in_alt ? dkey : dkey_alt, *v1 = in_alt ? gid : gid_alt;
        int alt2 = 0;
        GSR_HIP(onesweep_sort_pairs<uint32_t>(k0, v0, k1, v1, (uint32_t)N, 0, 32, depth_scratch, &alt2, st));
        sorted_gid = alt2 ? v1 : v0;
        launch_counts(BlendBalance{}, ZeroJobs{}, nullptr, ++pin.s->seq);
        GSR_HIP(hipStreamSynchronize(st));
        std::atomic_thread_fence(std::memory_order_acquire);
        R = *static_cast<volatile unsigned long long*>(pin.s->host);
        resorted = true;
    }
    if (R > 0xfffffff0ull) return fail(GSR_ERR_RANGE, "more than 2^32 instances%s");
    if (!speculative || R > cap || resorted) {
        if (speculative && !resorted) g_spec_overflows++;
        rc = alloc_binning(R);
        if (rc) return rc;
        rc = launch_binning(R, nullptr, false);
        if (rc) return rc;
        rc = launch_blend(false);
        if (rc) return rc;
    }
    {
        std::lock_guard<std::mutex> lk(g_state_mutex);
        uint64_t& h = g_hints[hint_key];
        h = std::max<uint64_t>(std::max<uint64_t>(R + R / 4, h - h / 32), 1u << 16);
        if (g_hints.size() > 4096) g_hints.clear();
    }
    out->num_rendered = (int64_t)R;
    if (ro) return GSR_OK;
    out->binning = bin;
    out->binning_bytes = B.bytes;
    out->binning_capacity = (int64_t)((speculative && R <= cap && !resorted) ? cap : R);
    out->forward_flags = pack_fwd_flags(opt_ppt, opt_map, opt_ckpt);
    return GSR_OK;
}

static int blend_bwd_resident(int has_da, int ppt = 2)
{
    static int cached[2][2] = {{0, 0}, {0, 0}};
    const int v = ppt == 1 ? 1 : 0;
    if (cached[v][has_da]) return cached[v][has_da];
    int dev = 0, cus = 256, per_cu = 0;
    hipDeviceProp_t prop;
    if (hipGetDevice(&dev) == hipSuccess && hipGetDeviceProperties(&prop, dev) == hipSuccess) cus = prop.multiProcessorCount;
    hipError_t e;
    if (v) e = has_da ? hipOccupancyMaxActiveBlocksPerMultiprocessor(&per_cu, k_blend_bwd1<true>, 256, 0)
                      : hipOccupancyMaxActiveBlocksPerMultiprocessor(&per_cu, k_blend_bwd1<false>, 256, 0);
    else e = has_da ? hipOccupancyMaxActiveBlocksPerMultiprocessor(&per_cu, k_blend_bwd2<true>, 128, 0)
                    : hipOccupancyMaxActiveBlocksPerMultiprocessor(&per_cu, k_blend_bwd2<false>, 128, 0);
    if (e != hipSuccess || per_cu < 1) per_cu = v ? 6 : 12;
    return cached[v][has_da] = per_cu * cus;
}

int gsr_backward(const GsrBackwardArgs* a, void* stream_)
{
    CallTimer call_timer(g_bwd_calls, g_bwd_ns);
    hipStream_t st = (hipStream_t)stream_;
    if (!a) return fail(GSR_ERR_ARG, "null args%s");
    if (a->forward_flags & GSR_FWD_FLAG_RENDER_ONLY)
        return fail(GSR_ERR_ARG, "gsr_backward: forward_flags come from a render-only forward, which keeps nothing a backward could read%s");
    int rc = check_common(a->N, a->M, a->D, a->W, a->H);
    if (rc) return rc;
    const int N = a->N, W = a->W, H = a->H;
    BatchDev bt;
    rc = batch_dev(a->batch, N, H, bt);
    if (rc) return rc;
    const int NB = bt.B;
    if (a->sh_origin && (!a->shs || NB > 1 || a->next_view))
        return fail(GSR_ERR_ARG, "sh_origin needs shs and is not served with a batch of B > 1 or a next_view%s");
    const bool want_cam = a->d_viewmatrix || a->d_projmatrix || a->d_campos || a->d_points_transform;
    const bool want_other_pg = a->d_opacities || a->d_colors_precomp || a->d_shs || a->d_shs_rest || a->d_scales || a->d_rotations || a->d_cov3D_precomp;
    const bool frozen = !a->fused_adam && !a->d_means3D && !want_other_pg && want_cam;
    if (!a->fused_adam && !a->d_means3D && a->N > 0) {
        if (want_other_pg)
            return fail(GSR_ERR_ARG, "d_means3D is NULL but another per-Gaussian gradient pointer is set: they come together, or none of them (frozen call)%s");
        if (!want_cam)
            return fail(GSR_ERR_ARG, "no gradient output: every per-Gaussian gradient pointer is NULL and so are d_viewmatrix, d_projmatrix, d_campos and "
                                     "d_points_transform%s");
        if (a->next_view || a->prepared_out)
            return fail(GSR_ERR_ARG, "a frozen call (no per-Gaussian gradient pointer) cannot prepare a next view: next_view / prepared_out need fused_adam%s");
        if (a->densify_stats)
            return fail(GSR_ERR_ARG, "a frozen call (no per-Gaussian gradient pointer) cannot accumulate densify_stats: they are fed by the per-Gaussian "
                                     "gradients it leaves out%s");
    }
    {
        int dev_id = 0;
        (void)hipGetDevice(&dev_id);
        unsigned long long got = 0, want = 0;
        bool bad = false;
        {
            std::lock_guard<std::mutex> lk(g_state_mutex);
            auto it = g_pin_slots.find(dev_id);
            if (it != g_pin_slots.end())
                for (PinSlot* s : it->second)
                    if (!s->busy && late_check(s, false, &got, &want)) { bad = true; break; }
        }
        if (bad) {
            char msg[200];
            snprintf(msg, sizeof msg, "a forward's binning was invalid: early instance count %llu, its scan counted %llu (or a sort look-back gave up)%%s", want, got);
            return fail(GSR_ERR_HIP, msg);
        }
    }
    int f_ppt = g_blend_ppt ? g_blend_ppt : 7, f_map = g_tile_map, f_ckpt = g_ckpt_first;
    if (a->forward_flags & 1) {
        f_ppt = (int)((a->forward_flags >> 1) & 7); f_map = (int)((a->forward_flags >> 4) & 3); f_ckpt = (int)((a->forward_flags >> 6) & 127);
        if (f_ppt < 1 || f_ppt > 7 || f_map > 2 || f_ckpt < 1) return fail(GSR_ERR_ARG, "forward_flags do not come from gsr_forward%s");
    }
    (void)f_ppt;
    if (N == 0) {
        if (a->d_viewmatrix) GSR_HIP(hipMemsetAsync(a->d_viewmatrix, 0, 64 * NB, st));
        if (a->d_projmatrix) GSR_HIP(hipMemsetAsync(a->d_projmatrix, 0, 64 * NB, st));
        if (a->d_campos) GSR_HIP(hipMemsetAsync(a->d_campos, 0, 12 * NB, st));
        if (a->d_points_transform) GSR_HIP(hipMemsetAsync(a->d_points_transform, 0, 48 * NB, st));
        return GSR_OK;
    }
    if (!a->geom || !a->image || !a->binning || !a->scratch || (!a->d_means2D && !frozen))
        return fail(GSR_ERR_ARG, "missing workspace / gradient pointer%s");
    const int tiles_x = (W + kTile - 1) / kTile, tiles_y = (H + kTile - 1) / kTile, T = tiles_x * tiles_y * NB;
    const Splat* splat = static_cast<const Splat*>(a->geom);
    BinLayout B = bin_layout(a->binning_capacity > 0 ? a->binning_capacity : a->num_rendered, W, H, NB);
    const uint8_t* bin = static_cast<const uint8_t*>(a->binning);
    const uint2* ranges = reinterpret_cast<const uint2*>(bin + B.ranges);
    const uint32_t* list = reinterpret_cast<const uint32_t*>(bin + B.list);
    double* gg = static_cast<double*>(a->scratch);
    uint32_t* prep_head = (a->next_view && a->prepared_out) ? reinterpret_cast<uint32_t*>(static_cast<uint8_t*>(a->prepared_out) + prep_layout(N).sort) : nullptr;
    bool prep_head_cleared = false;
    const int bwd_ppt = g_deterministic ? 2 : (g_bwd_ppt ? g_bwd_ppt : 2);
    const bool blend_items = a->num_rendered > 0;
    BwdItemHdr* item_hdr = nullptr;
    const uint2* items = nullptr;
    int bwd_grid = 0;
    {
        const uint32_t* staged4 = reinterpret_cast<const uint32_t*>(static_cast<const uint8_t*>(a->image) + image_staged_offset(W, H, NB));
        const int tpad = 8 * slots_per_xcd(f_map, T, tiles_x);
        const int want_split = g_bwd_split ? g_bwd_split : 16;
        const int split_ok = (want_split > 1 && f_ppt >= 5) ? 1 : 0;
        const size_t n4 = (size_t)N * kGG * sizeof(double) / sizeof(float4);
        int fill_blocks = (int)std::min<size_t>(4096, (n4 + 255) / 256);
        if (blend_items) {
            uint8_t* binw = const_cast<uint8_t*>(bin);
            item_hdr = reinterpret_cast<BwdItemHdr*>(binw + B.items);
            items = reinterpret_cast<const uint2*>(binw + B.items + kItemHdrBytes);
            const int64_t bound = (a->num_rendered >> 7) + T;
            const int resident = blend_bwd_resident((a->grad_depth || a->grad_alpha) ? 1 : 0, bwd_ppt);
            bwd_grid = (int)std::max<int64_t>(8, (std::min<int64_t>(resident, bound) + 7) / 8 * 8);
        }
        const uint32_t list_cap = (uint32_t)bwd_list_cap(a->binning_capacity > 0 ? a->binning_capacity : a->num_rendered, (size_t)T);
        hipLaunchKernelGGL(k_bwd_prologue, dim3(fill_blocks + (blend_items ? 8 : 0)), dim3(256), 0, st, reinterpret_cast<float4*>(gg), n4,
                           staged4, T, tiles_x, f_map, tpad, f_ckpt, split_ok, item_hdr, const_cast<uint2*>(items), list_cap,
                           (uint32_t)(bwd_grid / 8), blend_items ? prep_head : nullptr, (int)kOnesweepHeadWordsMax);
        prep_head_cleared = blend_items && prep_head != nullptr;
    }
    if (a->num_rendered > 0) {
        const int ppt = bwd_ppt;
        const float* img = static_cast<const float*>(a->image);
        ProfScope ps(P_BLEND_BWD, st);
        const float* ckpt = reinterpret_cast<const float*>(bin + B.ckpt);
        float* det_part = nullptr;
        uint8_t* det_mem = nullptr;
        const uint32_t Rn = (uint32_t)a->num_rendered;
        size_t o_part = 0, o_k0 = 0, o_k1 = 0, o_v0 = 0, o_v1 = 0, o_sort = 0, det_bytes = 0;
        if (g_deterministic) {
            size_t o = 0;
            o_part = o; o += align256((size_t)Rn * kDetStride * 4);
            o_k0 = o; o += align256((size_t)Rn * 4); o_k1 = o; o += align256((size_t)Rn * 4);
            o_v0 = o; o += align256((size_t)Rn * 4); o_v1 = o; o += align256((size_t)Rn * 4);
            o_sort = o; o += radix_scratch_bytes(Rn);
            det_bytes = o;
            GSR_HIP(hipMallocAsync((void**)&det_mem, det_bytes, st));
            det_part = reinterpret_cast<float*>(det_mem + o_part);
            GSR_HIP(hipMemsetAsync(det_part, 0, (size_t)Rn * kDetStride * 4, st));
        }
        BlendBwdArgs ba = {W, H, tiles_x, tiles_y, T, f_map, f_ckpt, 0, ranges, list, splat, a->bg, img, a->grad_color, a->grad_depth,
                           a->grad_alpha, gg, ckpt, det_part, item_hdr, items};
        if (ppt == 1) {
            if (a->grad_depth || a->grad_alpha) hipLaunchKernelGGL(k_blend_bwd1<true>, dim3(bwd_grid), dim3(256), 0, st, ba);
            else hipLaunchKernelGGL(k_blend_bwd1<false>, dim3(bwd_grid), dim3(256), 0, st, ba);
        } else if (a->grad_depth || a->grad_alpha) hipLaunchKernelGGL(k_blend_bwd2<true>, dim3(bwd_grid), dim3(128), 0, st, ba);
        else hipLaunchKernelGGL(k_blend_bwd2<false>, dim3(bwd_grid), dim3(128), 0, st, ba);
        if (g_deterministic) {
            uint32_t* k0 = reinterpret_cast<uint32_t*>(det_mem + o_k0); uint32_t* k1 = reinterpret_cast<uint32_t*>(det_mem + o_k1);
            uint32_t* v0 = reinterpret_cast<uint32_t*>(det_mem + o_v0); uint32_t* v1 = reinterpret_cast<uint32_t*>(det_mem + o_v1);
            hipLaunchKernelGGL(k_det_iota, dim3((Rn + 255) / 256), dim3(256), 0, st, Rn, v0, list, k0, (uint32_t)N);
            int nbits = 1;
            while ((1ll << nbits) < (long long)N) nbits++;
            int in_alt = 0;
            GSR_HIP(radix_sort_pairs<uint32_t>(k0, v0, k1, v1, Rn, 0, ((nbits + 7) / 8) * 8, det_mem + o_sort, &in_alt, st));
            hipLaunchKernelGGL(k_det_reduce, dim3((Rn + 255) / 256), dim3(256), 0, st, Rn, in_alt ? k1 : k0, in_alt ? v1 : v0, det_part, gg);
            GSR_HIP(hipFreeAsync(det_mem, st));
        }
    }
    CamParams cp = {a->viewmatrix, a->projmatrix, a->campos, a->tanfovx, a->tanfovy, a->scale_modifier, W, H, a->D, a->M, a->points_transform, bt};
    const int grid = (N + kPreThreads - 1) / kPreThreads;
    float* cam_partial = reinterpret_cast<float*>(static_cast<uint8_t*>(a->scratch) + align256((size_t)N * kGG * sizeof(double)));
    AdamDev ad = {};
    const GsrFusedAdam* fa = a->fused_adam;
    if (fa) {
        if (!a->raw_params || !a->shs || !a->shs_rest || a->cov3D_precomp || a->colors_precomp || !a->scales || !a->rotations || !a->opacities ||
            a->M < 1 || fa->step <= 0)
            return fail(GSR_ERR_ARG, "fused_adam needs raw_params with shs (f_dc) + shs_rest, scales, rotations and opacities%s");
        const bool skip_rest = !fa->exp_avg[2] && !fa->exp_avg_sq[2];
        if (skip_rest && (a->D != 0 || (a->next_view && a->next_view->D != 0)))
            return fail(GSR_ERR_ARG, "fused_adam: the f_rest group may be skipped only at sh_degree 0 (this render and the prepared one)%s");
        for (int q = 0; q < 6; q++) {
            ad.inv_bc2s[q] = 1.f;
            if (q == 2 && skip_rest) { ad.m[q] = nullptr; ad.v[q] = nullptr; ad.step_size[q] = 0.f; continue; }
            if (!fa->exp_avg[q] || !fa->exp_avg_sq[q]) return fail(GSR_ERR_ARG, "fused_adam: missing moment buffer%s");
            ad.m[q] = fa->exp_avg[q]; ad.v[q] = fa->exp_avg_sq[q];
            const int64_t tq = fa->step - (int64_t)fa->step_lag[q];
            if (fa->step_lag[q] < 0 || tq < 1) return fail(GSR_ERR_ARG, "fused_adam: step_lag out of range%s");
            ad.step_size[q] = fa->lr[q] / (float)(1.0 - pow((double)fa->beta1, (double)tq));
            ad.inv_bc2s[q] = 1.f / (float)sqrt(1.0 - pow((double)fa->beta2, (double)tq));
            const float* pin[6] = {a->means3D, a->shs, a->shs_rest, a->opacities, a->scales, a->rotations};
            if (fa->param_out[q] || fa->exp_avg_out[q] || fa->exp_avg_sq_out[q]) {
                if (!fa->param_out[q] || !fa->exp_avg_out[q] || !fa->exp_avg_sq_out[q]) return fail(GSR_ERR_ARG, "fused_adam: a group's three output buffers come together%s");
                if (a->next_view) return fail(GSR_ERR_ARG, "fused_adam: deferred application (param_out) cannot prepare a next view%s");
                ad.dp[q] = (long long)((const char*)fa->param_out[q] - (const char*)pin[q]);
                ad.dm[q] = (long long)((const char*)fa->exp_avg_out[q] - (const char*)fa->exp_avg[q]);
                ad.dv[q] = (long long)((const char*)fa->exp_avg_sq_out[q] - (const char*)fa->exp_avg_sq[q]);
            }
        }
        ad.b1 = fa->beta1; ad.b2 = fa->beta2; ad.eps = fa->eps;
    } else if (!frozen && (!a->d_means3D || !a->d_opacities))
        return fail(GSR_ERR_ARG, "missing workspace / gradient pointer%s");
    DensDev ds = {};
    if (a->densify_stats) {
        const GsrDensifyStats* q = a->densify_stats;
        if (!q->radii || !q->xyz_gradient_accum || !q->denom || !q->max_radii2D) return fail(GSR_ERR_ARG, "densify_stats: four pointers expected%s");
        ds.radii = q->radii; ds.grad_accum = q->xyz_gradient_accum; ds.denom = q->denom; ds.max_radii = q->max_radii2D;
    }
    PrepOut po = {};
    const GsrNextView* nv = a->next_view;
    if (nv) {
        if (!fa || !gsr_prepare_supported(a->M, a->D, a->raw_params) || nv->D < a->D || nv->D > a->D + 1 || nv->D > 3 || !a->prepared_out ||
            !nv->viewmatrix || !nv->projmatrix || !nv->campos || nv->W <= 0 || nv->H <= 0 ||
            ((((uintptr_t)a->shs | (uintptr_t)a->shs_rest) & 15) != 0))
            return fail(GSR_ERR_ARG, "next_view needs fused_adam, raw_params, M = 16, a next degree equal to this render's or one above, "
                                     "16-byte aligned SH tensors and a prepared_out buffer%s");
        const PrepLayout PL = prep_layout(N);
        uint8_t* pb = static_cast<uint8_t*>(a->prepared_out);
        BatchDev nbt = bt;
        if (NB > 1 && (long long)NB * ((nv->H + kTile - 1) / kTile) > 4095) return fail(GSR_ERR_RANGE, "batch: more than 4095 tile rows in the next view%s");
        po.cp = {nv->viewmatrix, nv->projmatrix, nv->campos, nv->tanfovx, nv->tanfovy, nv->scale_modifier, nv->W, nv->H, nv->D, a->M, nv->points_transform, nbt};
        po.splat = reinterpret_cast<Splat*>(pb + PL.splat);
        po.radii = reinterpret_cast<int32_t*>(pb + PL.radii);
        po.dkey = reinterpret_cast<uint32_t*>(pb + PL.dkey);
        po.gid = reinterpret_cast<uint32_t*>(pb + PL.gid);
        po.rec = reinterpret_cast<TileRec*>(pb + PL.rec);
        po.early_parts = reinterpret_cast<uint2*>(pb + PL.early);
        po.early_window = N > g_prep_hist_max_n ? (1u << 27) - 1u : 0xffffffffu;
        if (!prep_head_cleared) GSR_HIP(hipMemsetAsync(prep_head, 0, kOnesweepHeadWordsMax * sizeof(uint32_t), st));
        if (prep_counts_digits(N)) {
            po.dh.ghist = prep_head;
            po.dh.status = onesweep_status(pb + PL.sort);
            po.dh.status_words = onesweep_status_words<uint32_t>((uint32_t)N, 32);
            const int tail_blocks = ((N - (grid - 1) * kPreThreads) % 4 == 0) ? grid : grid - 1;
            po.dh.clear_threads = (uint32_t)tail_blocks * kPreThreads;
        }
    }
#define GSR_PREB_S(DEG, RAW, CAM, ADAM, PREP, SHO) GSR_PREB_SF(DEG, RAW, CAM, ADAM, PREP, SHO, false)
#define GSR_PREB_SF(DEG, RAW, CAM, ADAM, PREP, SHO, FROZEN)                                                                                 \
    hipLaunchKernelGGL((k_preprocess_bwd<DEG, RAW, CAM, ADAM, PREP, SHO, FROZEN>), dim3(grid), dim3(kPreThreads), 0, st, cp, N, a->means3D, \
                       a->scales, a->rotations, a->cov3D_precomp, a->shs, a->shs_rest, a->opacities, ad, splat, gg, a->d_means3D,           \
                       a->d_means2D, a->d_opacities, a->d_colors_precomp, a->d_shs, a->d_shs_rest, a->d_scales, a->d_rotations,             \
                       a->d_cov3D_precomp, cam_partial, po, ds, a->sh_origin)
#define GSR_PREB_(DEG, RAW, CAM, ADAM, PREP) GSR_PREB_S(DEG, RAW, CAM, ADAM, PREP, false)
#define GSR_PREB_SO(DEG, SHO)                                                                                                               \
    do {                                                                                                                                    \
        if (fa) { if (want_cam) GSR_PREB_S(DEG, true, true, true, -1, SHO); else GSR_PREB_S(DEG, true, false, true, -1, SHO); }             \
        else if (a->raw_params) { if (want_cam) GSR_PREB_S(DEG, true, true, false, -1, SHO); else GSR_PREB_S(DEG, true, false, false, -1, SHO); } \
        else { if (want_cam) GSR_PREB_S(DEG, false, true, false, -1, SHO); else GSR_PREB_S(DEG, false, false, false, -1, SHO); }           \
    } while (0)
#define GSR_PREB(DEG) GSR_PREB_SO(DEG, false)
#define GSR_PREB_FROZEN(DEG) do { if (a->raw_params) GSR_PREB_SF(DEG, true, true, false, -1, false, true); else GSR_PREB_SF(DEG, false, true, false, -1, false, true); } while (0)
#define GSR_PREB_NEXT(DEG, NDEG) do { if (want_cam) GSR_PREB_(DEG, true, true, true, NDEG); else GSR_PREB_(DEG, true, false, true, NDEG); } while (0)
#define GSR_PRE_TAIL(NDEG)                                                                                                               \
    hipLaunchKernelGGL((k_preprocess<NDEG, true>), dim3(1), dim3(kPreThreads), 0, st, po.cp, N, a->means3D, a->scales, a->rotations,       \
                       (const float*)nullptr, a->opacities, a->shs, a->shs_rest, (const float*)nullptr, po.splat, po.radii, po.dkey,     \
                       po.gid, po.rec, (uint32_t*)nullptr, 0, grid - 1, po.dh, po.early_parts, po.early_window)
    {
        ProfScope ps(P_PRE_BWD, st);
        if (nv) {
            switch (a->D * 4 + nv->D) {
                case 0: GSR_PREB_NEXT(0, 0); break;
                case 1: GSR_PREB_NEXT(0, 1); break;
                case 5: GSR_PREB_NEXT(1, 1); break;
                case 6: GSR_PREB_NEXT(1, 2); break;
                case 10: GSR_PREB_NEXT(2, 2); break;
                case 11: GSR_PREB_NEXT(2, 3); break;
                default: GSR_PREB_NEXT(3, 3); break;
            }
            const int nlast = N - (grid - 1) * kPreThreads;
            const bool last_lin = (nlast % 4) == 0;
            if (!last_lin) {
                switch (nv->D) {
                    case 0: GSR_PRE_TAIL(0); break;
                    case 1: GSR_PRE_TAIL(1); break;
                    case 2: GSR_PRE_TAIL(2); break;
                    default: GSR_PRE_TAIL(3); break;
                }
            }
        } else if (frozen) {
            g_frozen_bwd_calls.fetch_add(1, std::memory_order_relaxed);
            switch ((a->shs && !a->sh_origin) ? a->D : 0) {
                case 0: GSR_PREB_FROZEN(0); break;
                case 1: GSR_PREB_FROZEN(1); break;
                case 2: GSR_PREB_FROZEN(2); break;
                default: GSR_PREB_FROZEN(3); break;
            }
        } else if (a->sh_origin) {
        switch (a->D) {
            case 0: GSR_PREB(0); break;
            case 1: GSR_PREB_SO(1, true); break;
            case 2: GSR_PREB_SO(2, true); break;
            default: GSR_PREB_SO(3, true); break;
        }
        } else {
        switch (a->shs ? a->D : 0) {
            case 0: GSR_PREB(0); break;
            case 1: GSR_PREB(1); break;
            case 2: GSR_PREB(2); break;
            default: GSR_PREB(3); break;
        }
        }
    }
#undef GSR_PRE_TAIL
#undef GSR_PREB_NEXT
#undef GSR_PREB_FROZEN
#undef GSR_PREB
#undef GSR_PREB_SO
#undef GSR_PREB_
#undef GSR_PREB_SF
#undef GSR_PREB_S
    if (want_cam)
        hipLaunchKernelGGL(k_cam_reduce, dim3(kCamVals, NB), dim3(256), 0, st, cam_partial, grid, a->d_viewmatrix, a->d_projmatrix, a->d_campos,
                           a->d_points_transform, bt);
    GSR_HIP(hipGetLastError());
    return GSR_OK;
}

size_t gsr_importance_scratch_bytes(int32_t N) { return align256((size_t)(N > 0 ? N : 1) * kImpStride * sizeof(float)); }

int gsr_importance_accumulate(const GsrForwardArgs* a, const GsrForwardOut* out, float* acc, void* scratch, void* stream_)
{
    hipStream_t st = (hipStream_t)stream_;
    if (!a || !out) return fail(GSR_ERR_ARG, "null args%s");
    if (out->forward_flags & GSR_FWD_FLAG_RENDER_ONLY)
        return fail(GSR_ERR_ARG, "importance: forward_flags come from a render-only forward, which keeps no image state or lists for the pass%s");
    int rc = check_common(a->N, a->M, a->D, a->W, a->H);
    if (rc) return rc;
    if (a->colors_precomp || !a->shs) return fail(GSR_ERR_ARG, "importance: the model must carry SH coefficients (colors_precomp has none)%s");
    if (a->batch && a->batch->B > 1) return fail(GSR_ERR_ARG, "importance: not served with a batch of B > 1%s");
    if (a->M < (a->D + 1) * (a->D + 1) || !a->campos) return fail(GSR_ERR_ARG, "shs needs campos and M >= (D+1)^2%s");
    const int N = a->N, W = a->W, H = a->H;
    if (N == 0) return GSR_OK;
    if (!acc || !scratch || !a->geom || !a->image || !a->out_color || !a->means3D) return fail(GSR_ERR_ARG, "missing workspace / accumulator pointer%s");
    if (out->num_rendered <= 0 || !out->binning) return GSR_OK;
    int f_map = g_tile_map;
    if (out->forward_flags & 1) {
        f_map = (int)((out->forward_flags >> 4) & 3);
        if (f_map > 2) return fail(GSR_ERR_ARG, "forward_flags do not come from gsr_forward%s");
    }
// ... 18 lines not shown
                           a->sh_origin, splat, (const float*)S, acc);
    }
    GSR_HIP(hipGetLastError());
    return GSR_OK;
}

int gsr_debug_view_cache_stats(int32_t W, int32_t H, int64_t out[4])
{
    int dev_id = 0;
    if (hipGetDevice(&dev_id) != hipSuccess) return fail(GSR_ERR_HIP, "hipGetDevice failed%s");
    out[0] = out[1] = out[2] = out[3] = 0;
    std::vector<uint8_t*> mems;
    {
        std::lock_guard<std::mutex> lk(g_state_mutex);
        for (auto& c : g_view_costs) if (c.dev == dev_id && c.W == W && c.H == H) mems.push_back(c.mem);
    }
    for (uint8_t* m : mems) {
        ViewCostHdr h;
        if (hipDeviceSynchronize() != hipSuccess || hipMemcpy(&h, m, sizeof(h), hipMemcpyDeviceToHost) != hipSuccess)
            return fail(GSR_ERR_HIP, "view cache read-back failed%s");
        out[0] += h.pad[0]; out[1] += h.pad[1]; out[3] += 1;
        for (int i = 0; i < kVcEntries; i++) out[2] += h.key[i] != 0ull;
    }
    return GSR_OK;
}

int gsr_debug_list_cut_stats(int32_t W, int32_t H, int64_t out[5])
{
    int dev_id = 0;
    if (hipGetDevice(&dev_id) != hipSuccess) return fail(GSR_ERR_HIP, "hipGetDevice failed%s");
    out[0] = out[1] = out[2] = out[3] = out[4] = 0;
    std::vector<uint8_t*> mems;
    {
        std::lock_guard<std::mutex> lk(g_state_mutex);
        for (auto& c : g_view_costs) if (c.dev == dev_id && c.W == W && c.H == H) mems.push_back(c.mem);
    }
    for (uint8_t* m : mems) {
        ViewCostHdr h;
        if (hipDeviceSynchronize() != hipSuccess || hipMemcpy(&h, m, sizeof(h), hipMemcpyDeviceToHost) != hipSuccess)
            return fail(GSR_ERR_HIP, "view cache read-back failed%s");
        for (int q = 0; q < 5; q++) out[q] += h.pad[2 + q];
    }
    return GSR_OK;
}

int gsr_debug_direct_binning_geometry(int32_t N, int32_t T, int64_t out[7])
{
    if (!out) return GSR_ERR_ARG;
    DirectBin db = {};
    DirectBinScratch ds = {};
    const bool ok = direct_bin_geometry(N, T, db, ds);
    out[0] = ok ? 1 : 0; out[1] = db.S; out[2] = db.NC; out[3] = db.G; out[4] = db.Cg; out[5] = db.Tp; out[6] = ok ? (int64_t)ds.bytes : 0;
    return GSR_OK;
}

int gsr_debug_read_binning(const void* binning, int64_t binning_capacity, int64_t num_rendered, int32_t W, int32_t H,
                            uint32_t* ranges_out, uint32_t* list_out, void* stream_)
{
    if (!binning || W <= 0 || H <= 0 || num_rendered < 0) return fail(GSR_ERR_ARG, "bad debug_read_binning args%s");
    const BinLayout B = bin_layout(binning_capacity > 0 ? binning_capacity : num_rendered, W, H);
    const size_t T = (size_t)((W + kTile - 1) / kTile) * ((H + kTile - 1) / kTile);
    const uint8_t* bin = static_cast<const uint8_t*>(binning);
    hipStream_t st = (hipStream_t)stream_;
    if (ranges_out) GSR_HIP(hipMemcpyAsync(ranges_out, bin + B.ranges, T * sizeof(uint2), hipMemcpyDeviceToDevice, st));
    if (list_out && num_rendered > 0)
        GSR_HIP(hipMemcpyAsync(list_out, bin + B.list, (size_t)num_rendered * 4, hipMemcpyDeviceToDevice, st));
    return GSR_OK;
}

int64_t gsr_get_counter(const char* name)
{
    if (!name) return -1;
    if (!strcmp(name, "spec_overflows")) return g_spec_overflows.load();
    if (!strcmp(name, "late_checks")) return g_late_checks.load();
    if (!strcmp(name, "late_mismatches")) return g_late_mismatches.load();
    if (!strcmp(name, "depth_window_resorts")) return g_depth_window_resorts.load();
    if (!strcmp(name, "blend_bwd_resident")) return blend_bwd_resident(0);
    if (!strcmp(name, "spec_forwards")) return g_spec_forwards.load();
    if (!strcmp(name, "exact_forwards")) return g_exact_forwards.load();
    if (!strcmp(name, "forward_calls")) return g_fwd_calls.load();
    if (!strcmp(name, "forward_ns")) return g_fwd_ns.load();
    if (!strcmp(name, "forward_wait_ns")) return g_fwd_wait_ns.load();
    if (!strcmp(name, "backward_calls")) return g_bwd_calls.load();
    if (!strcmp(name, "backward_ns")) return g_bwd_ns.load();
    if (!strcmp(name, "frozen_backward_calls")) return g_frozen_bwd_calls.load();
    if (!strcmp(name, "spec_callers")) { std::lock_guard<std::mutex> lk(g_state_mutex); return (int64_t)g_hints.size(); }
    return -1;
}

int gsr_mark_visible(int32_t N, const float* means3D, const float* viewmatrix, const float* projmatrix, uint8_t* present, void* stream_)
{
    (void)projmatrix;
    if (N < 0 || (N > 0 && (!means3D || !viewmatrix || !present))) return fail(GSR_ERR_ARG, "bad mark_visible args%s");
    if (N == 0) return GSR_OK;
    hipLaunchKernelGGL(k_mark_visible, dim3((N + 255) / 256), dim3(256), 0, (hipStream_t)stream_, N, means3D, viewmatrix, present);
    GSR_HIP(hipGetLastError());
    return GSR_OK;
}

int gsr_sort_pairs_u32(uint32_t* keys, uint32_t* vals, uint32_t* keys_alt, uint32_t* vals_alt, uint32_t n, int begin_bit, int end_bit,
                       void* scratch, size_t scratch_bytes, int* result_in_alt, void* stream)
{
    if (scratch_bytes < radix_scratch_bytes(n) || !result_in_alt) return fail(GSR_ERR_ARG, "sort scratch too small%s");
    if (g_sort_algo && end_bit - begin_bit <= 32)
        GSR_HIP(onesweep_sort_pairs<uint32_t>(keys, vals, keys_alt, vals_alt, n, begin_bit, end_bit, scratch, result_in_alt, (hipStream_t)stream));
    else
        GSR_HIP(radix_sort_pairs<uint32_t>(keys, vals, keys_alt, vals_alt, n, begin_bit, end_bit, scratch, result_in_alt, (hipStream_t)stream));
    return GSR_OK;
}

int gsr_sort_pairs_u16(uint16_t* keys, uint32_t* vals, uint16_t* keys_alt, uint32_t* vals_alt, uint32_t n, int begin_bit, int end_bit,
                       void* scratch, size_t scratch_bytes, int* result_in_alt, void* stream)
{
    if (scratch_bytes < radix_scratch_bytes(n) || !result_in_alt) return fail(GSR_ERR_ARG, "sort scratch too small%s");
    if (g_sort_algo)
        GSR_HIP(onesweep_sort_pairs<uint16_t>(keys, vals, keys_alt, vals_alt, n, begin_bit, end_bit, scratch, result_in_alt, (hipStream_t)stream));
    else
        GSR_HIP(radix_sort_pairs<uint16_t>(keys, vals, keys_alt, vals_alt, n, begin_bit, end_bit, scratch, result_in_alt, (hipStream_t)stream));
    return GSR_OK;
}

}
```

### 3dgs_hierarchical_training_amd/csrc/radix_sort.h

```cpp
#pragma once
#include <map>
#include <mutex>
#include <utility>
#include <hip/hip_runtime.h>
#include <stdint.h>

namespace gsr {

constexpr int kSortThreads = 256;
constexpr int kSortIPT = 16;
constexpr int kSortTile = kSortThreads * kSortIPT;
constexpr int kSortWaves = kSortThreads / 64;

__device__ __forceinline__ unsigned long long lanemask_lt()
{
    const unsigned lane = __builtin_amdgcn_mbcnt_hi(~0u, __builtin_amdgcn_mbcnt_lo(~0u, 0u));
    return (1ull << lane) - 1ull;
}

template <int IPT, int NB = 256>
__device__ __forceinline__ void wave_rank(unsigned long long* s_mask, uint32_t* s_cnt, const uint32_t (&dig)[IPT],
                                          uint32_t (&rnk)[IPT], int lane)
{
#pragma unroll
// ... 55 lines not shown
    if (base + kSortTile <= n && (((uintptr_t)(keys + base)) & 15) == 0) {
        constexpr int KPV = 16 / (int)sizeof(KeyT);
        constexpr int NV = kSortTile / KPV / kSortThreads;
        const uint4* v4 = reinterpret_cast<const uint4*>(keys + base);
#pragma unroll
        for (int r = 0; r < NV; r++) {
            const uint4 q = v4[r * kSortThreads + tid];
            const uint32_t w[4] = {q.x, q.y, q.z, q.w};
#pragma unroll
            for (int c = 0; c < 4; c++) {
                if (sizeof(KeyT) == 4) atomicAdd(&h[(w[c] >> shift) & 0xffu], 1u);
                else {
                    atomicAdd(&h[((w[c] & 0xffffu) >> shift) & 0xffu], 1u);
                    atomicAdd(&h[((w[c] >> 16) >> shift) & 0xffu], 1u);
                }
            }
        }
    } else {
#pragma unroll
        for (int r = 0; r < kSortIPT; r++) {
            const uint32_t idx = base + r * kSortThreads + tid;
            if (idx < n) atomicAdd(&h[((uint32_t)keys[idx] >> shift) & 0xffu], 1u);
        }
    }
    __syncthreads();
    hist[(uint32_t)tid * nblocks + blockIdx.x] = h[tid];
    if (h[tid]) atomicAdd(&totals[tid], h[tid]);
}

static __global__ __launch_bounds__(256) void k_radix_scan(uint32_t* __restrict__ hist, uint32_t nblocks,
                                                    const uint32_t* __restrict__ totals)
{
    __shared__ uint32_t s_part[256];
    const int tid = threadIdx.x;
    const int d = blockIdx.x;
    uint32_t digit_base = 0;
    for (int k = 0; k < d; k++) digit_base += totals[k];
    uint32_t* row = hist + (size_t)d * nblocks;
    const uint32_t chunk = (nblocks + 255u) / 256u;
    const uint32_t lo = min(nblocks, (uint32_t)tid * chunk), hi = min(nblocks, lo + chunk);
    uint32_t sum = 0;
    for (uint32_t b = lo; b < hi; b++) sum += row[b];
    s_part[tid] = sum;
    __syncthreads();
    for (int off = 1; off < 256; off <<= 1) {
        uint32_t v = (tid >= off) ? s_part[tid - off] : 0u;
        __syncthreads();
        s_part[tid] += v;
        __syncthreads();
    }
    uint32_t run = digit_base + s_part[tid] - sum;
    for (uint32_t b = lo; b < hi; b++) {
        const uint32_t c = row[b];
        row[b] = run;
        run += c;
    }
}

template <typename KeyT>
__global__ __launch_bounds__(kSortThreads) void k_radix_scatter(const KeyT* __restrict__ kin, const uint32_t* __restrict__ vin,
                                                                KeyT* __restrict__ kout, uint32_t* __restrict__ vout, uint32_t n,
                                                                int shift, const uint32_t* __restrict__ hist, uint32_t nblocks)
{
    __shared__ unsigned long long s_mask[kSortWaves][256];
    __shared__ uint32_t s_cnt[kSortWaves][256];
    __shared__ KeyT s_keys[kSortTile];
    __shared__ uint32_t s_vals[kSortTile];
    __shared__ uint32_t s_start[256];
    __shared__ uint32_t s_gbase[256];
    __shared__ uint32_t s_wsum[kSortWaves];
    const int tid = threadIdx.x, wave = tid >> 6, lane = tid & 63;
    const uint32_t base = blockIdx.x * (uint32_t)kSortTile;
    const uint32_t valid = min((uint32_t)kSortTile, n - base);

    KeyT key[kSortIPT];
    uint32_t val[kSortIPT];
    uint32_t dig[kSortIPT];
    uint32_t rnk[kSortIPT];
#pragma unroll
    for (int r = 0; r < kSortIPT; r++) {
        const uint32_t p = (uint32_t)(wave * (kSortIPT * 64) + r * 64 + lane);
        if (p < valid) {
            key[r] = kin[base + p];
            val[r] = vin[base + p];
            dig[r] = ((uint32_t)key[r] >> shift) & 0xffu;
        } else {
            key[r] = (KeyT)~(KeyT)0; val[r] = 0u; dig[r] = 255u;
        }
    }
    wave_rank<kSortIPT>(s_mask[wave], s_cnt[wave], dig, rnk, lane);
    __syncthreads();
    uint32_t mine = 0;
#pragma unroll
    for (int w = 0; w < kSortWaves; w++) {
        const uint32_t c = s_cnt[w][tid];
        s_cnt[w][tid] = mine;
        mine += c;
    }
    const uint32_t excl = block_scan_excl<kSortWaves>(mine, s_wsum, tid);
    s_start[tid] = excl;
    s_gbase[tid] = hist[(size_t)tid * nblocks + blockIdx.x] - excl;
    __syncthreads();
#pragma unroll
    for (int r = 0; r < kSortIPT; r++) {
        const uint32_t lp = s_start[dig[r]] + s_cnt[wave][dig[r]] + rnk[r];
        s_keys[lp] = key[r];
        s_vals[lp] = val[r];
    }
    __syncthreads();
#pragma unroll
    for (int r = 0; r < kSortIPT; r++) {
        const uint32_t p = r * kSortThreads + tid;
        if (p < valid) {
            const KeyT k = s_keys[p];
            const uint32_t d = ((uint32_t)k >> shift) & 0xffu;
            const uint32_t g = s_gbase[d] + p;
            kout[g] = k;
            vout[g] = s_vals[p];
        }
    }
}

template <typename KeyT> struct OsCfg { static constexpr int kThreads = 512, kTile = 5120; };
template <> struct OsCfg<uint32_t> { static constexpr int kThreads = 1024, kTile = 4096; };

template <typename KernelT>
inline uint32_t onesweep_resident_blocks(KernelT kernel, int threads)
{
    static std::mutex mu;
    static std::map<std::pair<int, const void*>, uint32_t> cache;
    int dev = 0;
    if (hipGetDevice(&dev) != hipSuccess) return 0;
    const auto key = std::make_pair(dev, reinterpret_cast<const void*>(kernel));
    std::lock_guard<std::mutex> lk(mu);
    auto it = cache.find(key);
    if (it != cache.end()) return it->second;
    int per_cu = 0, cus = 0;
    uint32_t v = 0;
    if (hipOccupancyMaxActiveBlocksPerMultiprocessor(&per_cu, kernel, threads, 0) == hipSuccess &&
        hipDeviceGetAttribute(&cus, hipDeviceAttributeMultiprocessorCount, dev) == hipSuccess && per_cu > 0 && cus > 0)
        v = (uint32_t)per_cu * (uint32_t)cus;
    cache[key] = v;
    return v;
}
__device__ unsigned int g_onesweep_giveups = 0u;
struct OsRider;
constexpr int kOsRanges = 32;
constexpr uint32_t kOsLocal = 1u << 30, kOsIncl = 2u << 30, kOsMask = (1u << 30) - 1u;
constexpr uint32_t kOsTicketWords = (4 * kOsRanges + 63) / 64 * 64;
constexpr uint32_t kOnesweepHeadWords = 4 * kOsRanges * 256 + kOsTicketWords;
constexpr uint32_t kOnesweepHeadWords9 = 3 * kOsRanges * 512 + kOsTicketWords;
constexpr uint32_t kOnesweepHeadWordsMax = kOnesweepHeadWords9 > kOnesweepHeadWords ? kOnesweepHeadWords9 : kOnesweepHeadWords;
inline unsigned int* onesweep_overflow_word(void* scratch) { return static_cast<unsigned int*>(scratch) + 3 * kOsRanges * 512 + 100; }

template <typename KeyT>
__host__ __device__ inline uint32_t onesweep_run_len(uint32_t n)
{
    constexpr uint64_t kT = (uint64_t)OsCfg<KeyT>::kTile;
    const uint64_t ntiles = ((uint64_t)n + kT - 1) / kT, per = (ntiles + kOsRanges - 1) / kOsRanges;
    return (uint32_t)(per * kT);
}
__host__ __device__ inline int onesweep_passes(int bits) { return (bits + 7) / 8; }
__host__ __device__ inline int onesweep_dbits(int bits) { const int p = onesweep_passes(bits); return (bits + p - 1) / p; }
template <typename KeyT>
__host__ __device__ inline uint32_t onesweep_status_words(uint32_t capacity, int bits)
{
    const uint32_t nblocks = (capacity + OsCfg<KeyT>::kTile - 1) / OsCfg<KeyT>::kTile;
// ... 108 lines not shown
        uint2 v[8];
#pragma unroll
        for (int u = 0; u < 8; u++) {
            const uint32_t q = q0 + (uint32_t)u * blockDim.x;
            v[u] = q < rd.nparts ? rd.parts[q] : make_uint2(0u, 0u);
        }
#pragma unroll
        for (int u = 0; u < 8; u++) { a += v[u].x; b += v[u].y; }
    }
#pragma unroll
    for (int off = 32; off > 0; off >>= 1) { a += __shfl_xor(a, off, 64); b += __shfl_xor(b, off, 64); }
    if ((threadIdx.x & 63u) == 0u) { s_r[0][threadIdx.x >> 6] = a; s_r[1][threadIdx.x >> 6] = b; }
    __syncthreads();
    if (threadIdx.x == 0) {
        a = b = 0ull;
        for (uint32_t w = 0; w < blockDim.x / 64u; w++) { a += s_r[0][w]; b += s_r[1][w]; }
        __atomic_store_n(rd.host + 2, (unsigned long long)g_onesweep_giveups, __ATOMIC_RELAXED);
        __atomic_store_n(rd.host + 3, b, __ATOMIC_RELAXED);
        __atomic_store_n(rd.host, a, __ATOMIC_RELAXED);
        __threadfence_system();
        __atomic_store_n(rd.host + 1, rd.seq, __ATOMIC_RELAXED);
        __threadfence_system();
    }
}

constexpr int kOsTile = 4096;

#ifdef GSR_OS_TIMING
__device__ unsigned long long g_os_dbg[4096 * 8];
#define OS_T(k) do { const unsigned long long now_ = __builtin_readcyclecounter(); if (threadIdx.x == 0) ost[k] += now_ - ost_last; ost_last = now_; } while (0)
#else
#define OS_T(k) do { } while (0)
#endif
template <typename KeyT, int NB>
__global__ __launch_bounds__(OsCfg<KeyT>::kThreads) void k_onesweep(const KeyT* __restrict__ kin, const uint32_t* __restrict__ vin,
                                                         KeyT* __restrict__ kout, uint32_t* __restrict__ vout, uint32_t n, int shift,
                                                         const uint32_t* __restrict__ ghist ,
                                                         uint32_t* __restrict__ status ,
                                                         uint32_t* __restrict__ ticket,
                                                         const unsigned long long* __restrict__ n_dev, uint32_t dmask, int runs,
                                                         uint32_t bias = 0u, uint32_t kclamp = 0xffffffffu, OsRider rider = OsRider{})
{
    constexpr int GS = NB > 256 ? NB : 256;
    constexpr int kOsThreads = OsCfg<KeyT>::kThreads, kOsTile = OsCfg<KeyT>::kTile, kOsIPT = kOsTile / kOsThreads, kOsWaves = kOsThreads / 64;
    if (rider.host && blockIdx.x == gridDim.x - 1) {
        __shared__ unsigned long long s_r[2][16];
        onesweep_rider_publish(rider, s_r);
    }
    if (n_dev) n = (uint32_t)min((unsigned long long)n, *n_dev);
    __shared__ unsigned long long s_mask[kOsWaves][NB];
    __shared__ uint32_t s_cnt[kOsWaves][NB];
    __shared__ KeyT s_keys[kOsTile];
    __shared__ uint32_t s_vals[kOsTile];
    __shared__ uint32_t s_start[NB];
    __shared__ uint32_t s_gbase[NB];
    __shared__ uint32_t s_wsum[kOsWaves];
    __shared__ uint32_t s_tile;
    const int tid = threadIdx.x, wave = tid >> 6, lane = tid & 63;
#ifdef GSR_OS_TIMING
    unsigned long long ost[8] = {0, 0, 0, 0, 0, 0, 0, 0}, ost_last = __builtin_readcyclecounter();
    ost[6] = ost_last;
#endif
    const uint32_t ntiles = (uint32_t)(((uint64_t)n + kOsTile - 1) / kOsTile);
    const uint32_t per = runs > 1 ? (ntiles + kOsRanges - 1) / kOsRanges : ntiles;
    const uint32_t run = runs > 1 ? (blockIdx.x & (kOsRanges - 1)) : 0u;
    uint32_t krun = runs > 1 ? blockIdx.x / kOsRanges : blockIdx.x;
    if (ticket) {
        if (tid == 0) s_tile = atomicAdd(ticket + run, 1u);
        __syncthreads();
        krun = s_tile;
    }
    const uint32_t run_start = run * per;
    const uint32_t tile = run_start + krun;
    if (krun >= per || tile >= ntiles) return;
    const uint32_t base = tile * (uint32_t)kOsTile;
    const uint32_t valid = min((uint32_t)kOsTile, n - base);
    KeyT key[kOsIPT];
    uint32_t val[kOsIPT], dig[kOsIPT], rnk[kOsIPT];
#pragma unroll
    for (int r = 0; r < kOsIPT; r++) {
        const uint32_t p = (uint32_t)(wave * (kOsIPT * 64) + r * 64 + lane);
        if (p < valid) {
            key[r] = kin[base + p];
            val[r] = vin[base + p];
            dig[r] = (min((uint32_t)key[r] - bias, kclamp) >> shift) & dmask;
        } else {
            key[r] = (KeyT)~(KeyT)0; val[r] = 0u; dig[r] = (uint32_t)(NB - 1);
        }
    }
    OS_T(0);
    wave_rank<kOsIPT, NB>(s_mask[wave], s_cnt[wave], dig, rnk, lane);
    __syncthreads();
    OS_T(1);
    const bool is_digit = tid < NB;
    uint32_t mine = 0;
    if (is_digit) {
#pragma unroll
        for (int w = 0; w < kOsWaves; w++) {
            const uint32_t c = s_cnt[w][tid];
            s_cnt[w][tid] = mine;
            mine += c;
        }
    }
    const uint32_t real = (tid == NB - 1) ? mine - ((uint32_t)kOsTile - valid) : mine;
    uint32_t* my_status = status + (size_t)tile * GS + (tid & (NB - 1));
    if (is_digit) __hip_atomic_store(my_status, kOsLocal | real, __ATOMIC_RELAXED, __HIP_MEMORY_SCOPE_AGENT);
    const uint32_t lstart = block_scan_excl<kOsWaves>(mine, s_wsum, tid);
    uint32_t gtot = 0u, gpre = 0u;
    if (is_digit) {
#pragma unroll
        for (int x = 0; x < kOsRanges; x++) {
            const uint32_t c = ghist[x * GS + tid];
            gtot += c;
            gpre += (uint32_t)x < run ? c : 0u;
        }
    }
    const uint32_t dbase = block_scan_excl<kOsWaves>(gtot, s_wsum, tid) + gpre;
    OS_T(2);
    if (is_digit) {
        uint32_t excl = 0, polls = 0;
        const int t_lo = (int)run_start;
        for (int t = (int)tile - 1; t >= t_lo;) {
            constexpr int kWin = 4;
            uint32_t v[kWin];
#pragma unroll
            for (int q = 0; q < kWin; q++)
                v[q] = (t - q >= t_lo) ? __hip_atomic_load(status + (size_t)(t - q) * GS + tid, __ATOMIC_RELAXED, __HIP_MEMORY_SCOPE_AGENT) : kOsIncl;
            bool done = false;
#pragma unroll
            for (int q = 0; q < kWin; q++) {
                if (done) break;
                const uint32_t f = v[q] & ~kOsMask;
                if (f == 0u) { done = true; break; }
                excl += v[q] & kOsMask;
                t--;
                if (f == kOsIncl) { t = t_lo - 1; done = true; }
            }
            if (t >= t_lo && done) {
                __builtin_amdgcn_s_sleep(1);
                if (++polls > (1u << 23)) { atomicAdd(&g_onesweep_giveups, 1u); break; }
            }
        }
        __hip_atomic_store(my_status, kOsIncl | (excl + real), __ATOMIC_RELAXED, __HIP_MEMORY_SCOPE_AGENT);
        s_start[tid] = lstart;
        s_gbase[tid] = dbase + excl - lstart;
    }
    __syncthreads();
    OS_T(3);
#pragma unroll
    for (int r = 0; r < kOsIPT; r++) {
        const uint32_t lp = s_start[dig[r]] + s_cnt[wave][dig[r]] + rnk[r];
        s_keys[lp] = key[r];
        s_vals[lp] = val[r];
    }
    __syncthreads();
    OS_T(4);
#pragma unroll
    for (int r = 0; r < kOsIPT; r++) {
        const uint32_t p = r * kOsThreads + tid;
        if (p < valid) {
            const KeyT k = s_keys[p];
            const uint32_t d = (min((uint32_t)k - bias, kclamp) >> shift) & dmask;
            const uint32_t g = s_gbase[d] + p;
            kout[g] = k;
            vout[g] = s_vals[p];
        }
    }
#ifdef GSR_OS_TIMING
    OS_T(5);
    if (tid == 0 && sizeof(KeyT) == 4 && blockIdx.x < 4096) { ost[7] = ost_last; for (int q = 0; q < 8; q++) g_os_dbg[blockIdx.x * 8 + q] = ost[q]; }
#endif
}

inline size_t onesweep_scratch_bytes(uint32_t n)
{
    const size_t nblocks = ((size_t)n + kOsTile - 1) / kOsTile;
    const size_t nb = nblocks ? nblocks : 1;
    const size_t w8 = kOnesweepHeadWords + 4 * nb * 256, w9 = kOnesweepHeadWords9 + 3 * nb * 512;
    return ((w8 > w9 ? w8 : w9) * sizeof(uint32_t) + 255) & ~(size_t)255;
}

template <typename KeyT>
inline hipError_t onesweep_sort_pairs(KeyT* keys, uint32_t* vals, KeyT* keys_alt, uint32_t* vals_alt, uint32_t n, int begin_bit,
                                      int end_bit, void* scratch, int* in_alt, hipStream_t stream,
                                      const unsigned long long* n_dev = nullptr, bool head_prezeroed = false, bool hist_done = false,
                                      int max_digit_bits = 8, uint32_t bias = 0u, const OsRider* rider = nullptr)
{
    const bool wide_ = max_digit_bits == 9;
    const OsRider rd = (rider && (wide_ || !hist_done)) ? *rider : OsRider{};
    const OsRider rd0 = (rider && !wide_ && hist_done) ? *rider : OsRider{};
    *in_alt = 0;
    if (n == 0) return hipSuccess;
    const int bits = end_bit - begin_bit;
    const bool wide = max_digit_bits == 9;
    const int passes = (bits + (wide ? 9 : 8) - 1) / (wide ? 9 : 8);
    if (passes < 1 || passes > 4 || (wide && (passes != 3 || sizeof(KeyT) != 4 || hist_done || begin_bit != 0))) return hipErrorInvalidValue;
    const uint32_t GS = wide ? 512u : 256u;
    const uint32_t kclamp = (wide && bits < 32) ? ((1u << bits) - 1u) : 0xffffffffu;
    if (!wide) bias = 0u;
    const int dbits = (bits + passes - 1) / passes;
    const uint32_t nblocks = (n + OsCfg<KeyT>::kTile - 1) / OsCfg<KeyT>::kTile;
    uint32_t* ghist = static_cast<uint32_t*>(scratch);
    uint32_t* tickets = ghist + (wide ? 3 * kOsRanges * 512 : 4 * kOsRanges * 256);
    uint32_t* status = tickets + kOsTicketWords;
    if (!head_prezeroed && !hist_done) {
        hipError_t e = hipMemsetAsync(scratch, 0, (wide ? kOnesweepHeadWords9 : kOnesweepHeadWords) * sizeof(uint32_t), stream);
        if (e != hipSuccess) return e;
    }
    const uint32_t status_words = (uint32_t)((size_t)passes * nblocks * GS);
    const uint32_t per_cap = (nblocks + kOsRanges - 1) / kOsRanges;
    const uint32_t hgrid = kOsRanges * (per_cap < 32u ? per_cap : 32u);
    if (wide)
        hipLaunchKernelGGL((k_radix_ghist<KeyT, 3, 512>), dim3(hgrid), dim3(256), 0, stream, keys, n, begin_bit, ghist, n_dev, status, status_words, dbits, bits,
                           bias, kclamp, onesweep_overflow_word(scratch), rd);
    else if (!hist_done)
    switch (passes) {
        case 1: hipLaunchKernelGGL((k_radix_ghist<KeyT, 1>), dim3(hgrid), dim3(256), 0, stream, keys, n, begin_bit, ghist, n_dev, status, status_words, dbits, bits, 0u, 0xffffffffu, (unsigned int*)nullptr, rd); break;
        case 2: hipLaunchKernelGGL((k_radix_ghist<KeyT, 2>), dim3(hgrid), dim3(256), 0, stream, keys, n, begin_bit, ghist, n_dev, status, status_words, dbits, bits, 0u, 0xffffffffu, (unsigned int*)nullptr, rd); break;
        case 3: hipLaunchKernelGGL((k_radix_ghist<KeyT, 3>), dim3(hgrid), dim3(256), 0, stream, keys, n, begin_bit, ghist, n_dev, status, status_words, dbits, bits, 0u, 0xffffffffu, (unsigned int*)nullptr, rd); break;
        default: hipLaunchKernelGGL((k_radix_ghist<KeyT, 4>), dim3(hgrid), dim3(256), 0, stream, keys, n, begin_bit, ghist, n_dev, status, status_words, dbits, bits, 0u, 0xffffffffu, (unsigned int*)nullptr, rd); break;
    }
    KeyT *kin = keys, *kout = keys_alt;
    uint32_t *vin = vals, *vout = vals_alt;
    for (int p = 0; p < passes; p++) {
        const uint32_t pmask = (1u << (dbits < bits - dbits * p ? dbits : bits - dbits * p)) - 1u;
        const int runs = p == 0 ? kOsRanges : 1;
        const uint32_t pgrid = runs > 1 ? kOsRanges * per_cap : nblocks;
        const int wbits = dbits < bits - dbits * p ? dbits : bits - dbits * p;
        const uint32_t resident = wbits <= 6 ? onesweep_resident_blocks(k_onesweep<KeyT, 64>, OsCfg<KeyT>::kThreads)
                                             : onesweep_resident_blocks(k_onesweep<KeyT, 256>, OsCfg<KeyT>::kThreads);
        uint32_t* tk_p = pgrid <= resident ? (uint32_t*)nullptr : tickets + p * kOsRanges;
        if (wide) {
            const uint32_t res9 = onesweep_resident_blocks(k_onesweep<KeyT, 512>, OsCfg<KeyT>::kThreads);
            uint32_t* tk9 = pgrid <= res9 ? (uint32_t*)nullptr : tickets + p * kOsRanges;
            hipLaunchKernelGGL((k_onesweep<KeyT, 512>), dim3(pgrid), dim3(OsCfg<KeyT>::kThreads), 0, stream, kin, vin, kout, vout, n,
                               begin_bit + dbits * p, ghist + p * kOsRanges * 512, status + (size_t)p * nblocks * 512, tk9, n_dev, pmask, runs, bias, kclamp);
        } else if (wbits <= 6)
            hipLaunchKernelGGL((k_onesweep<KeyT, 64>), dim3(pgrid), dim3(OsCfg<KeyT>::kThreads), 0, stream, kin, vin, kout, vout, n,
                               begin_bit + dbits * p, ghist + p * kOsRanges * 256, status + (size_t)p * nblocks * 256, tk_p, n_dev, pmask, runs,
                               0u, 0xffffffffu, p == 0 ? rd0 : OsRider{});
        else
            hipLaunchKernelGGL((k_onesweep<KeyT, 256>), dim3(pgrid), dim3(OsCfg<KeyT>::kThreads), 0, stream, kin, vin, kout, vout, n,
                               begin_bit + dbits * p, ghist + p * kOsRanges * 256, status + (size_t)p * nblocks * 256, tk_p, n_dev, pmask, runs,
                               0u, 0xffffffffu, p == 0 ? rd0 : OsRider{});
        KeyT* tk = kin; kin = kout; kout = tk;
        uint32_t* tv = vin; vin = vout; vout = tv;
        *in_alt ^= 1;
    }
    return hipGetLastError();
}

inline size_t radix_scratch_bytes(uint32_t n)
{
    const size_t nblocks = ((size_t)n + kSortTile - 1) / kSortTile;
    const size_t osblocks = ((size_t)n + kOsTile - 1) / kOsTile;
    const size_t three_kernel = ((256 * (nblocks ? nblocks : 1) + 8 * 256) * sizeof(uint32_t) + 255) & ~(size_t)255;
    const size_t onesweep = onesweep_scratch_bytes(n);
    (void)osblocks;
    return three_kernel > onesweep ? three_kernel : onesweep;
}

template <typename KeyT>
inline hipError_t radix_sort_pairs(KeyT* keys, uint32_t* vals, KeyT* keys_alt, uint32_t* vals_alt, uint32_t n, int begin_bit,
                                   int end_bit, void* scratch, int* in_alt, hipStream_t stream)
{
    *in_alt = 0;
    if (n == 0) return hipSuccess;
    const uint32_t nblocks = (n + kSortTile - 1) / kSortTile;
    uint32_t* hist = static_cast<uint32_t*>(scratch);
    uint32_t* totals = hist + (size_t)256 * nblocks;
    hipError_t e = hipMemsetAsync(totals, 0, 8 * 256 * sizeof(uint32_t), stream);
    if (e != hipSuccess) return e;
    KeyT *kin = keys, *kout = keys_alt;
    uint32_t *vin = vals, *vout = vals_alt;
    for (int shift = begin_bit; shift < end_bit; shift += 8, totals += 256) {
        hipLaunchKernelGGL(k_radix_hist<KeyT>, dim3(nblocks), dim3(kSortThreads), 0, stream, kin, n, shift, hist, nblocks, totals);
        hipLaunchKernelGGL(k_radix_scan, dim3(256), dim3(256), 0, stream, hist, nblocks, totals);
        hipLaunchKernelGGL(k_radix_scatter<KeyT>, dim3(nblocks), dim3(kSortThreads), 0, stream, kin, vin, kout, vout, n, shift,
                           hist, nblocks);
        KeyT* tk = kin; kin = kout; kout = tk;
        uint32_t* tv = vin; vin = vout; vout = tv;
        *in_alt ^= 1;
    }
    return hipGetLastError();
}

}
```

Measured before the change: 1258.

## Generate sort values as iota, skip final key write, fold grad clear into blend

```diff
diff --git a/3dgs_hierarchical_training_amd/csrc/gsr_kernels.hip b/3dgs_hierarchical_training_amd/csrc/gsr_kernels.hip
--- a/3dgs_hierarchical_training_amd/csrc/gsr_kernels.hip
+++ b/3dgs_hierarchical_training_amd/csrc/gsr_kernels.hip
@@ -377,7 +377,7 @@
                                                             const float* __restrict__ shs, const float* __restrict__ shs_rest,
                                                             const float* __restrict__ colors,
                                                             Splat* __restrict__ splat, int32_t* __restrict__ radii,
-                                                            uint32_t* __restrict__ dkey, uint32_t* __restrict__ gid,
+                                                            uint32_t* __restrict__ dkey,
                                                             TileRec* __restrict__ tilerec, uint32_t* __restrict__ zero_words,
                                                             int zero_count, int block0, DepthHist dh, uint2* __restrict__ early_parts = nullptr,
                                                             uint32_t window_max = 0xffffffffu, uint8_t* __restrict__ visible = nullptr,
@@ -513,7 +513,6 @@
     if (visible) visible[i] = s.radius > 0 ? 1 : 0;
     const uint32_t key = s.tiles > 0 ? __float_as_uint(s.depth) : 0xffffffffu;
     dkey[i] = key;
-    gid[i] = (uint32_t)i;
     if (dh.ghist) {
         const uint32_t x = (uint32_t)i / onesweep_run_len<uint32_t>((uint32_t)N);
 #pragma unroll
@@ -2163,23 +2162,28 @@
 }
 
 
-constexpr size_t kItemHdrBytes = 2048;
+constexpr int kClearShards = 64;
+constexpr size_t kItemHdrStruct = 2048;
+constexpr size_t kItemHdrBytes = kItemHdrStruct + (size_t)kClearShards * 128;
 struct BwdItemHdr {
     uint32_t count[8];
     uint32_t offset[8];
     uint32_t pad[16];
     uint32_t head[8][32];
 };
-static_assert(sizeof(BwdItemHdr) <= kItemHdrBytes, "item header");
+static_assert(sizeof(BwdItemHdr) <= kItemHdrStruct, "item header");
 constexpr int kItemBuckets = 32;
 
 __global__ __launch_bounds__(256) void k_bwd_prologue(float4* __restrict__ gg4, size_t n4, const uint32_t* __restrict__ staged4, int T,
                                                       int tiles_x, int interleave, int tpad, int kCkptFirst, int split_ok,
                                                       BwdItemHdr* __restrict__ hdr, uint2* __restrict__ items, uint32_t list_cap,
-                                                      uint32_t first_pull, uint32_t* __restrict__ zero_words, int zero_count)
+                                                      uint32_t first_pull, uint32_t* __restrict__ zero_words, int zero_count,
+                                                      uint32_t* __restrict__ clear_done = nullptr)
 {
     const int tid = threadIdx.x;
     const int builders = hdr ? 8 : 0;
+    if (clear_done && blockIdx.x == 0)
+        for (int q = tid; q < kClearShards * 32; q += 256) clear_done[q] = 0u;
     if ((int)blockIdx.x >= builders) {
         const size_t nblk = gridDim.x - builders, blk = blockIdx.x - builders;
         const float4 z = {0.f, 0.f, 0.f, 0.f};
@@ -2239,6 +2243,9 @@
     float* det_part;
     BwdItemHdr* hdr;
     const uint2* items;
+    float4* clear4;
+    unsigned long long clear_n4;
+    uint32_t* clear_done;
 };
 
 #ifdef GSR_K8_PHASES
@@ -2247,6 +2254,33 @@
 #else
 #define K8_T(k) do { } while (0)
 #endif
+__device__ __noinline__ void bwd_clear_slice(float4* c4, unsigned long long n4, uint32_t* done)
+{
+    const unsigned long long per = (n4 + gridDim.x - 1) / gridDim.x;
+    const unsigned long long lo = min(n4, per * blockIdx.x), hi = min(n4, lo + per);
+    const float4 z = {0.f, 0.f, 0.f, 0.f};
+    for (unsigned long long i = lo + threadIdx.x; i < hi; i += blockDim.x) nt_store4(c4 + i, z);
+    __builtin_amdgcn_fence(__ATOMIC_RELEASE, "agent");
+    __syncthreads();
+    if (threadIdx.x == 0) __hip_atomic_fetch_add(done + (blockIdx.x & (kClearShards - 1)) * 32u, 1u, __ATOMIC_RELEASE, __HIP_MEMORY_SCOPE_AGENT);
+}
+__device__ __noinline__ void bwd_clear_wait(const uint32_t* done)
+{
+    if (threadIdx.x < 64u) {
+        const uint32_t* const mine = done + threadIdx.x * 32u;
+        for (uint32_t polls = 0;;) {
+            uint32_t c = __hip_atomic_load(mine, __ATOMIC_RELAXED, __HIP_MEMORY_SCOPE_AGENT);
+#pragma unroll
+            for (int off = 32; off > 0; off >>= 1) c += (uint32_t)__shfl_xor((int)c, off, 64);
+            if (c >= gridDim.x) break;
+            __builtin_amdgcn_s_sleep(8);
+            if (++polls > (1u << 23)) { if (threadIdx.x == 0) atomicAdd(&g_onesweep_giveups, 1u); break; }
+        }
+    }
+    __syncthreads();
+    __builtin_amdgcn_fence(__ATOMIC_ACQUIRE, "agent");
+}
+
 template <bool HAS_DA>
 __global__ __launch_bounds__(128) void k_blend_bwd2(BlendBwdArgs args_)
 {
@@ -2264,6 +2298,11 @@
     constexpr float kL2E = 1.4426950408889634f, kLn2 = 0.6931471805599453f;
 #pragma unroll
     for (int k = 0; k < NV; k++) s_part[threadIdx.x][k] = 0.f;
+    bool cleared = true;
+    if (args_.clear4) {
+        bwd_clear_slice(args_.clear4, args_.clear_n4, args_.clear_done);
+        cleared = false;
+    }
     int qx = (int)(blockIdx.x & 7u), tried = 0;
     uint32_t qi = blockIdx.x >> 3;
     for (;;) {
@@ -2505,6 +2544,10 @@
         K8_T(3);
         __syncthreads();
         K8_T(4);
+        if (!cleared) {
+            bwd_clear_wait(ka->clear_done);
+            cleared = true;
+        }
         {
             const int r = tid & 15, q = tid >> 4;
             for (int jj = q; jj < cnt; jj += NT / 16) {
@@ -2808,7 +2851,6 @@
     Splat* splat;
     int32_t* radii;
     uint32_t* dkey;
-    uint32_t* gid;
     TileRec* rec;
     DepthHist dh;
     uint2* early_parts;
@@ -3428,7 +3470,6 @@
                 po.radii[i] = s2.radius;
                 key2 = s2.tiles > 0 ? __float_as_uint(s2.depth) : 0xffffffffu;
                 po.dkey[i] = key2;
-                po.gid[i] = (uint32_t)i;
             }
             K9_T(4);
             if (po.dh.ghist) {
@@ -3582,7 +3623,7 @@
 }
 
 struct PrepLayout {
-    size_t splat, radii, dkey, gid, rec, sort, early, bytes;
+    size_t splat, radii, dkey, rec, sort, early, bytes;
 };
 static PrepLayout prep_layout(int32_t N)
 {
@@ -3592,7 +3633,6 @@
     p.splat = o; o += align256(n * sizeof(Splat));
     p.radii = o; o += align256(n * 4);
     p.dkey = o; o += align256(n * 4);
-    p.gid = o; o += align256(n * 4);
     p.rec = o; o += align256(n * sizeof(TileRec));
     p.sort = o; o += align256(onesweep_scratch_bytes((uint32_t)n));
     p.early = o; o += align256(((n + kPreThreads - 1) / kPreThreads) * sizeof(uint2));
@@ -3668,6 +3708,7 @@
 static std::map<std::tuple<int, int, int, int>, uint64_t> g_hints;
 static long long g_hint_override = -1;
 static int g_speculate = 1;
+static int g_bwd_clear_in_blend = 0;
 static int g_deterministic = 0;
 static int g_bwd_split = 0;
 static int g_ckpt_first = 1;
@@ -3685,7 +3726,7 @@
 static int g_blend_balance = 1;
 static int g_tile_map = 2;
 static std::atomic<long long> g_spec_overflows{0}, g_spec_forwards{0}, g_exact_forwards{0}, g_depth_window_resorts{0};
-static std::atomic<long long> g_fwd_calls{0}, g_fwd_ns{0}, g_fwd_wait_ns{0}, g_bwd_calls{0}, g_bwd_ns{0}, g_frozen_bwd_calls{0};
+static std::atomic<long long> g_fwd_calls{0}, g_fwd_ns{0}, g_fwd_wait_ns{0}, g_bwd_calls{0}, g_bwd_ns{0}, g_frozen_bwd_calls{0}, g_bwd_clears_in_blend{0};
 struct CallTimer {
     std::atomic<long long>&calls, &ns;
     std::chrono::steady_clock::time_point t0 = std::chrono::steady_clock::now();
@@ -3871,6 +3912,7 @@
         g_blend_ppt = value; return GSR_OK;
     }
     if (!strcmp(name, "ab_variants")) return 0;
+    if (!strcmp(name, "bwd_clear_in_blend")) { g_bwd_clear_in_blend = value ? 1 : 0; return GSR_OK; }
     if (!strcmp(name, "bwd_split")) { if (value < 0 || value > 64) return GSR_ERR_ARG; g_bwd_split = value; return GSR_OK; }
     if (!strcmp(name, "ckpt_first")) { if (value < 1 || value > 64) return GSR_ERR_ARG; g_ckpt_first = value; return GSR_OK; }
     if (!strcmp(name, "tile_map")) { if (value < 0 || value > 2) return GSR_ERR_ARG; g_tile_map = value; return GSR_OK; }
@@ -4239,7 +4281,6 @@
         const PrepLayout PL = prep_layout(N);
         uint8_t* pb = static_cast<uint8_t*>(a->prepared);
         dkey = reinterpret_cast<uint32_t*>(pb + PL.dkey);
-        gid = reinterpret_cast<uint32_t*>(pb + PL.gid);
         ntiles = reinterpret_cast<TileRec*>(pb + PL.rec);
         ProfScope ps(P_PRE_FWD, st);
         if (depth_onesweep) { depth_scratch = pb + PL.sort; depth_hist_done = prep_counts_digits(N); }
@@ -4249,7 +4290,7 @@
     } else {
 #define GSR_PRE_(DEG, RAW, SHO)                                                                                                     \
     hipLaunchKernelGGL((k_preprocess<DEG, RAW, SHO>), dim3(grid), dim3(kPreThreads), 0, st, cp, N, a->means3D, a->scales,           \
-                       a->rotations, a->cov3D_precomp, a->opacities, a->shs, a->shs_rest, a->colors_precomp, splat, a->radii, dkey, gid, \
+                       a->rotations, a->cov3D_precomp, a->opacities, a->shs, a->shs_rest, a->colors_precomp, splat, a->radii, dkey, \
                        ntiles, zero_words, zero_count, 0, DepthHist{}, early_parts, early_window, a->visible, a->sh_origin)
 #define GSR_PRE(DEG) do { if (a->raw_params) GSR_PRE_(DEG, true, false); else GSR_PRE_(DEG, false, false); } while (0)
 #define GSR_PRE_SHO(DEG) do { if (a->raw_params) GSR_PRE_(DEG, true, true); else GSR_PRE_(DEG, false, true); } while (0)
@@ -4298,11 +4339,13 @@
     OsRider rider = {};
     if (early_r) { rider.parts = early_parts; rider.nparts = (uint32_t)grid; rider.host = pin.s->dev; rider.seq = ++pin.s->seq; }
     ts_rec = ntiles; ts_dkey = dkey;
+    const bool depth_keys_wanted = !depth_onesweep || g_list_cut == 2 || (g_list_cut == 1 && N >= g_list_cut_min_n);
     if (!tsort) {
         ProfScope ps(P_SORT_DEPTH, st);
         GSR_HIP(depth_onesweep ? onesweep_sort_pairs<uint32_t>(dkey, gid, dkey_alt, gid_alt, (uint32_t)N, 0, wide_depth ? 27 : 32, depth_scratch, &in_alt, st,
-                                                               nullptr, true, depth_hist_done, wide_depth ? 9 : 8, kDepthKeyBias, early_r ? &rider : nullptr)
-                               : radix_sort_pairs<uint32_t>(dkey, gid, dkey_alt, gid_alt, (uint32_t)N, 0, 32, fs + L.sort, &in_alt, st));
+                                                               nullptr, true, depth_hist_done, wide_depth ? 9 : 8, kDepthKeyBias, early_r ? &rider : nullptr,
+                                                               kOsIotaVals | (depth_keys_wanted ? 0 : kOsValsOnly))
+                               : radix_sort_pairs<uint32_t>(dkey, gid, dkey_alt, gid_alt, (uint32_t)N, 0, 32, fs + L.sort, &in_alt, st, true));
     }
     sorted_gid = tsort ? nullptr : (in_alt ? gid_alt : gid);
     auto launch_counts = [&](const BlendBalance& bal, const ZeroJobs& zjobs, const unsigned int* wo, unsigned long long seq, bool publish = true) {
@@ -4366,7 +4409,7 @@
                     bb.vm = a->viewmatrix; bb.pt = a->points_transform; bb.view_id = (long long)a->view_id;
                     bb.tol = 1e-6f * (float)g_view_pose_tol_e6;
                     bb.items = items; bb.nslots4 = nslots4; bb.W = W; bb.H = H;
-                    if (!ro && direct && !tsort && db.NC <= 16000 && T == db.T && (g_list_cut == 2 || (g_list_cut == 1 && N >= g_list_cut_min_n))) {
+                    if (!ro && depth_keys_wanted && direct && !tsort && db.NC <= 16000 && T == db.T && (g_list_cut == 2 || (g_list_cut == 1 && N >= g_list_cut_min_n))) {
                         uint8_t* dm = fs + align256(L.bytes);
                         lc.key = reinterpret_cast<uint32_t*>(mem + vc_cut);
                         lc.owner_n = reinterpret_cast<uint32_t*>(mem + vc_own);
@@ -4438,7 +4481,7 @@
             seen = gv;
         }
         if (fresh)
-            return fail(GSR_ERR_HIP, "a radix-sort look-back gave up (status words overwritten?): the binning of this or the previous forward is invalid%s");
+            return fail(GSR_ERR_HIP, "a radix-sort look-back gave up (status words overwritten?): the binning of this or the previous forward is invalid -- or the backward blend's wait for its accumulator clear did (\"bwd_clear_in_blend\"): the previous backward's gradients are%s");
         if (early_r) {
             pin.s->pending = true; pin.s->pending_seq = rider.seq; pin.s->pending_R = R + (unsigned long long)g_debug_late_bias; pin.s->pending_giveups = gv;
             g_debug_late_bias = 0;
@@ -4448,7 +4491,8 @@
     if (wide_depth && static_cast<volatile unsigned long long*>(pin.s->host)[3] != 0ull) {
         { std::lock_guard<std::mutex> lk(g_state_mutex); g_full_depth_sort[hint_key] = true; }
         g_depth_window_resorts++;
-        uint32_t *k0 = in_alt ? dkey_alt : dkey, *v0 = in_alt ? gid_alt : gid, *k1 = in_alt ? dkey : dkey_alt, *v1 = in_alt ? gid : gid_alt;
+        const int src_alt = depth_keys_wanted ? in_alt : in_alt ^ 1;
+        uint32_t *k0 = src_alt ? dkey_alt : dkey, *v0 = src_alt ? gid_alt : gid, *k1 = src_alt ? dkey : dkey_alt, *v1 = src_alt ? gid : gid_alt;
         int alt2 = 0;
         GSR_HIP(onesweep_sort_pairs<uint32_t>(k0, v0, k1, v1, (uint32_t)N, 0, 32, depth_scratch, &alt2, st));
         sorted_gid = alt2 ? v1 : v0;
@@ -4483,6 +4527,7 @@
     return GSR_OK;
 }
 
+static bool g_bwd_resident_asked[2][2] = {{false, false}, {false, false}};
 static int blend_bwd_resident(int has_da, int ppt = 2)
 {
     static int cached[2][2] = {{0, 0}, {0, 0}};
@@ -4496,6 +4541,7 @@
                       : hipOccupancyMaxActiveBlocksPerMultiprocessor(&per_cu, k_blend_bwd1<false>, 256, 0);
     else e = has_da ? hipOccupancyMaxActiveBlocksPerMultiprocessor(&per_cu, k_blend_bwd2<true>, 128, 0)
                     : hipOccupancyMaxActiveBlocksPerMultiprocessor(&per_cu, k_blend_bwd2<false>, 128, 0);
+    g_bwd_resident_asked[v][has_da] = e == hipSuccess && per_cu >= 1;
     if (e != hipSuccess || per_cu < 1) per_cu = v ? 6 : 12;
     return cached[v][has_da] = per_cu * cus;
 }
@@ -4578,6 +4624,7 @@
     BwdItemHdr* item_hdr = nullptr;
     const uint2* items = nullptr;
     int bwd_grid = 0;
+    uint32_t* clear_in_blend = nullptr;
     {
         const uint32_t* staged4 = reinterpret_cast<const uint32_t*>(static_cast<const uint8_t*>(a->image) + image_staged_offset(W, H, NB));
         const int tpad = 8 * slots_per_xcd(f_map, T, tiles_x);
@@ -4585,6 +4632,7 @@
         const int split_ok = (want_split > 1 && f_ppt >= 5) ? 1 : 0;
         const size_t n4 = (size_t)N * kGG * sizeof(double) / sizeof(float4);
         int fill_blocks = (int)std::min<size_t>(4096, (n4 + 255) / 256);
+        uint32_t* clear_done = nullptr;
         if (blend_items) {
             uint8_t* binw = const_cast<uint8_t*>(bin);
             item_hdr = reinterpret_cast<BwdItemHdr*>(binw + B.items);
@@ -4592,11 +4640,18 @@
             const int64_t bound = (a->num_rendered >> 7) + T;
             const int resident = blend_bwd_resident((a->grad_depth || a->grad_alpha) ? 1 : 0, bwd_ppt);
             bwd_grid = (int)std::max<int64_t>(8, (std::min<int64_t>(resident, bound) + 7) / 8 * 8);
+            if (g_bwd_clear_in_blend && bwd_ppt == 2 && !g_deterministic && want_split > 1 && bwd_grid <= resident &&
+                g_bwd_resident_asked[0][(a->grad_depth || a->grad_alpha) ? 1 : 0] && n4 <= (size_t)bwd_grid * 4096) {
+                clear_done = reinterpret_cast<uint32_t*>(binw + B.items + kItemHdrStruct);
+                fill_blocks = 0;
+                g_bwd_clears_in_blend++;
+            }
         }
         const uint32_t list_cap = (uint32_t)bwd_list_cap(a->binning_capacity > 0 ? a->binning_capacity : a->num_rendered, (size_t)T);
         hipLaunchKernelGGL(k_bwd_prologue, dim3(fill_blocks + (blend_items ? 8 : 0)), dim3(256), 0, st, reinterpret_cast<float4*>(gg), n4,
                            staged4, T, tiles_x, f_map, tpad, f_ckpt, split_ok, item_hdr, const_cast<uint2*>(items), list_cap,
-                           (uint32_t)(bwd_grid / 8), blend_items ? prep_head : nullptr, (int)kOnesweepHeadWordsMax);
+                           (uint32_t)(bwd_grid / 8), blend_items ? prep_head : nullptr, (int)kOnesweepHeadWordsMax, clear_done);
+        clear_in_blend = clear_done;
         prep_head_cleared = blend_items && prep_head != nullptr;
     }
     if (a->num_rendered > 0) {
@@ -4620,7 +4675,9 @@
             GSR_HIP(hipMemsetAsync(det_part, 0, (size_t)Rn * kDetStride * 4, st));
         }
         BlendBwdArgs ba = {W, H, tiles_x, tiles_y, T, f_map, f_ckpt, 0, ranges, list, splat, a->bg, img, a->grad_color, a->grad_depth,
-                           a->grad_alpha, gg, ckpt, det_part, item_hdr, items};
+                           a->grad_alpha, gg, ckpt, det_part, item_hdr, items,
+                           clear_in_blend ? reinterpret_cast<float4*>(gg) : nullptr, (unsigned long long)((size_t)N * kGG * sizeof(double) / sizeof(float4)),
+                           clear_in_blend};
         if (ppt == 1) {
             if (a->grad_depth || a->grad_alpha) hipLaunchKernelGGL(k_blend_bwd1<true>, dim3(bwd_grid), dim3(256), 0, st, ba);
             else hipLaunchKernelGGL(k_blend_bwd1<false>, dim3(bwd_grid), dim3(256), 0, st, ba);
@@ -4693,7 +4750,6 @@
         po.splat = reinterpret_cast<Splat*>(pb + PL.splat);
         po.radii = reinterpret_cast<int32_t*>(pb + PL.radii);
         po.dkey = reinterpret_cast<uint32_t*>(pb + PL.dkey);
-        po.gid = reinterpret_cast<uint32_t*>(pb + PL.gid);
         po.rec = reinterpret_cast<TileRec*>(pb + PL.rec);
         po.early_parts = reinterpret_cast<uint2*>(pb + PL.early);
         po.early_window = N > g_prep_hist_max_n ? (1u << 27) - 1u : 0xffffffffu;
@@ -4725,7 +4781,7 @@
 #define GSR_PRE_TAIL(NDEG)                                                                                                               \
     hipLaunchKernelGGL((k_preprocess<NDEG, true>), dim3(1), dim3(kPreThreads), 0, st, po.cp, N, a->means3D, a->scales, a->rotations,       \
                        (const float*)nullptr, a->opacities, a->shs, a->shs_rest, (const float*)nullptr, po.splat, po.radii, po.dkey,     \
-                       po.gid, po.rec, (uint32_t*)nullptr, 0, grid - 1, po.dh, po.early_parts, po.early_window)
+                       po.rec, (uint32_t*)nullptr, 0, grid - 1, po.dh, po.early_parts, po.early_window)
     {
         ProfScope ps(P_PRE_BWD, st);
         if (nv) {
@@ -4910,6 +4966,7 @@
     if (!strcmp(name, "forward_ns")) return g_fwd_ns.load();
     if (!strcmp(name, "forward_wait_ns")) return g_fwd_wait_ns.load();
     if (!strcmp(name, "backward_calls")) return g_bwd_calls.load();
+    if (!strcmp(name, "bwd_clears_in_blend")) return g_bwd_clears_in_blend.load();
     if (!strcmp(name, "backward_ns")) return g_bwd_ns.load();
     if (!strcmp(name, "frozen_backward_calls")) return g_frozen_bwd_calls.load();
     if (!strcmp(name, "spec_callers")) { std::lock_guard<std::mutex> lk(g_state_mutex); return (int64_t)g_hints.size(); }
diff --git a/3dgs_hierarchical_training_amd/csrc/radix_sort.h b/3dgs_hierarchical_training_amd/csrc/radix_sort.h
--- a/3dgs_hierarchical_training_amd/csrc/radix_sort.h
+++ b/3dgs_hierarchical_training_amd/csrc/radix_sort.h
@@ -161,7 +161,7 @@
         const uint32_t p = (uint32_t)(wave * (kSortIPT * 64) + r * 64 + lane);
         if (p < valid) {
             key[r] = kin[base + p];
-            val[r] = vin[base + p];
+            val[r] = vin ? vin[base + p] : base + p;
             dig[r] = ((uint32_t)key[r] >> shift) & 0xffu;
         } else {
             key[r] = (KeyT)~(KeyT)0; val[r] = 0u; dig[r] = 255u;
@@ -436,7 +436,7 @@
         const uint32_t p = (uint32_t)(wave * (kOsIPT * 64) + r * 64 + lane);
         if (p < valid) {
             key[r] = kin[base + p];
-            val[r] = vin[base + p];
+            val[r] = vin ? vin[base + p] : base + p;
             dig[r] = (min((uint32_t)key[r] - bias, kclamp) >> shift) & dmask;
         } else {
             key[r] = (KeyT)~(KeyT)0; val[r] = 0u; dig[r] = (uint32_t)(NB - 1);
@@ -516,7 +516,7 @@
             const KeyT k = s_keys[p];
             const uint32_t d = (min((uint32_t)k - bias, kclamp) >> shift) & dmask;
             const uint32_t g = s_gbase[d] + p;
-            kout[g] = k;
+            if (kout) kout[g] = k;
             vout[g] = s_vals[p];
         }
     }
@@ -534,11 +534,12 @@
     return ((w8 > w9 ? w8 : w9) * sizeof(uint32_t) + 255) & ~(size_t)255;
 }
 
+constexpr int kOsIotaVals = 1, kOsValsOnly = 2;
 template <typename KeyT>
 inline hipError_t onesweep_sort_pairs(KeyT* keys, uint32_t* vals, KeyT* keys_alt, uint32_t* vals_alt, uint32_t n, int begin_bit,
                                       int end_bit, void* scratch, int* in_alt, hipStream_t stream,
                                       const unsigned long long* n_dev = nullptr, bool head_prezeroed = false, bool hist_done = false,
-                                      int max_digit_bits = 8, uint32_t bias = 0u, const OsRider* rider = nullptr)
+                                      int max_digit_bits = 8, uint32_t bias = 0u, const OsRider* rider = nullptr, int trims = 0)
 {
     const bool wide_ = max_digit_bits == 9;
     const OsRider rd = (rider && (wide_ || !hist_done)) ? *rider : OsRider{};
@@ -579,6 +580,8 @@
     for (int p = 0; p < passes; p++) {
         const uint32_t pmask = (1u << (dbits < bits - dbits * p ? dbits : bits - dbits * p)) - 1u;
         const int runs = p == 0 ? kOsRanges : 1;
+        const uint32_t* vin_p = (p == 0 && (trims & kOsIotaVals)) ? (const uint32_t*)nullptr : vin;
+        KeyT* kout_p = (p == passes - 1 && (trims & kOsValsOnly)) ? (KeyT*)nullptr : kout;
         const uint32_t pgrid = runs > 1 ? kOsRanges * per_cap : nblocks;
         const int wbits = dbits < bits - dbits * p ? dbits : bits - dbits * p;
         const uint32_t resident = wbits <= 6 ? onesweep_resident_blocks(k_onesweep<KeyT, 64>, OsCfg<KeyT>::kThreads)
@@ -587,14 +590,14 @@
         if (wide) {
             const uint32_t res9 = onesweep_resident_blocks(k_onesweep<KeyT, 512>, OsCfg<KeyT>::kThreads);
             uint32_t* tk9 = pgrid <= res9 ? (uint32_t*)nullptr : tickets + p * kOsRanges;
-            hipLaunchKernelGGL((k_onesweep<KeyT, 512>), dim3(pgrid), dim3(OsCfg<KeyT>::kThreads), 0, stream, kin, vin, kout, vout, n,
+            hipLaunchKernelGGL((k_onesweep<KeyT, 512>), dim3(pgrid), dim3(OsCfg<KeyT>::kThreads), 0, stream, kin, vin_p, kout_p, vout, n,
                                begin_bit + dbits * p, ghist + p * kOsRanges * 512, status + (size_t)p * nblocks * 512, tk9, n_dev, pmask, runs, bias, kclamp);
         } else if (wbits <= 6)
-            hipLaunchKernelGGL((k_onesweep<KeyT, 64>), dim3(pgrid), dim3(OsCfg<KeyT>::kThreads), 0, stream, kin, vin, kout, vout, n,
+            hipLaunchKernelGGL((k_onesweep<KeyT, 64>), dim3(pgrid), dim3(OsCfg<KeyT>::kThreads), 0, stream, kin, vin_p, kout_p, vout, n,
                                begin_bit + dbits * p, ghist + p * kOsRanges * 256, status + (size_t)p * nblocks * 256, tk_p, n_dev, pmask, runs,
                                0u, 0xffffffffu, p == 0 ? rd0 : OsRider{});
         else
-            hipLaunchKernelGGL((k_onesweep<KeyT, 256>), dim3(pgrid), dim3(OsCfg<KeyT>::kThreads), 0, stream, kin, vin, kout, vout, n,
+            hipLaunchKernelGGL((k_onesweep<KeyT, 256>), dim3(pgrid), dim3(OsCfg<KeyT>::kThreads), 0, stream, kin, vin_p, kout_p, vout, n,
                                begin_bit + dbits * p, ghist + p * kOsRanges * 256, status + (size_t)p * nblocks * 256, tk_p, n_dev, pmask, runs,
                                0u, 0xffffffffu, p == 0 ? rd0 : OsRider{});
         KeyT* tk = kin; kin = kout; kout = tk;
@@ -616,7 +619,7 @@
 
 template <typename KeyT>
 inline hipError_t radix_sort_pairs(KeyT* keys, uint32_t* vals, KeyT* keys_alt, uint32_t* vals_alt, uint32_t n, int begin_bit,
-                                   int end_bit, void* scratch, int* in_alt, hipStream_t stream)
+                                   int end_bit, void* scratch, int* in_alt, hipStream_t stream, bool iota_vals = false)
 {
     *in_alt = 0;
     if (n == 0) return hipSuccess;
@@ -630,7 +633,8 @@
     for (int shift = begin_bit; shift < end_bit; shift += 8, totals += 256) {
         hipLaunchKernelGGL(k_radix_hist<KeyT>, dim3(nblocks), dim3(kSortThreads), 0, stream, kin, n, shift, hist, nblocks, totals);
         hipLaunchKernelGGL(k_radix_scan, dim3(256), dim3(256), 0, stream, hist, nblocks, totals);
-        hipLaunchKernelGGL(k_radix_scatter<KeyT>, dim3(nblocks), dim3(kSortThreads), 0, stream, kin, vin, kout, vout, n, shift,
+        hipLaunchKernelGGL(k_radix_scatter<KeyT>, dim3(nblocks), dim3(kSortThreads), 0, stream, kin,
+                           (iota_vals && shift == begin_bit) ? (const uint32_t*)nullptr : vin, kout, vout, n, shift,
                            hist, nblocks);
         KeyT* tk = kin; kin = kout; kout = tk;
         uint32_t* tv = vin; vin = vout; vout = tv;
```

Result: no change. 1248 (-0.8%).
